# vsois/hanabi-agents

Hardware: AMD Instinct MI355X
Metric: env_steps_per_sec (higher is better)
Workload: dtype u8 env/encoder + bfloat16 Q-net GEMM (fp32 accumulate, fp32 master weights)

## Files before the change

### hanabi-agents_amd/csrc/actor_fused.hip

```cpp
#include <hip/hip_runtime.h>
#include <hip/hip_bf16.h>
#include <hip/hip_fp16.h>

#include <cstdint>

#include "../../include/hanabi_hip.h"
#include "common.hpp"
#include "env_kernel.hpp"

using hb::fail;

namespace {

typedef __bf16 bf16x8 __attribute__((ext_vector_type(8)));
typedef _Float16 f16x8 __attribute__((ext_vector_type(8)));
typedef float f32x4 __attribute__((ext_vector_type(4)));

constexpr int FM = 128;
constexpr int FH = 512;
constexpr int FNT = 512;
constexpr int FK = 51;
constexpr int S2 = FH / 32;
constexpr int LUT_BYTES = 65536;
constexpr int H_BYTES = FM * FH * 2;
constexpr int FRAG_FLOATS = 3 * 8 * FM;
constexpr int LDS_TOTAL = H_BYTES + FRAG_FLOATS * 4;
constexpr float NEG_BIG = -1e30f;

struct FusedArgs {
  const uint32_t* obs;
  long long m;
  int words;
  int s1;
  const uint4* w1f;
  const float* b1;
  const uint4* w2f;
  const float* b2;
  const float* support;
  float* q;
  int n_actions, n_pass;
  const int8_t* legal;
  int32_t* actions;
  float epsilon;
  unsigned long long seed, draw;
  long long first_gid;
  unsigned long long* stamps;
};

#ifdef HB_STAMPS
#define HB_FSTAMP(slot)                                                                              \
  do {                                                                                               \
    __builtin_amdgcn_sched_barrier(0);                                                               \
    unsigned long long hb_t_;                                                                        \
    asm volatile("s_memtime %0\n\ts_waitcnt lgkmcnt(0)" : "=s"(hb_t_)::"memory");                    \
    if (a.stamps && lane == 0) a.stamps[(static_cast<long long>(blockIdx.x) * 8 + wave) * 16 + (slot)] = hb_t_; \
    __builtin_amdgcn_sched_barrier(0);                                                               \
  } while (0)
#define HB_FSTAMP_REAL(slot)                                                                         \
  do {                                                                                               \
    unsigned long long hb_t_;                                                                        \
    asm volatile("s_memrealtime %0\n\ts_waitcnt lgkmcnt(0)" : "=s"(hb_t_)::"memory");                \
    if (a.stamps && lane == 0) a.stamps[(static_cast<long long>(blockIdx.x) * 8 + wave) * 16 + (slot)] = hb_t_; \
  } while (0)
#else
#define HB_FSTAMP(slot) do {} while (0)
#define HB_FSTAMP_REAL(slot) do {} while (0)
#endif

template <bool F16>
__device__ __forceinline__ uint32_t pack16(float lo, float hi) {
  if constexpr (F16) {
    const _Float16 a = static_cast<_Float16>(lo), b = static_cast<_Float16>(hi);
    uint16_t ua, ub;
    __builtin_memcpy(&ua, &a, 2);
    __builtin_memcpy(&ub, &b, 2);
    return static_cast<uint32_t>(ua) | (static_cast<uint32_t>(ub) << 16);
  } else {
    const __hip_bfloat16 a = __float2bfloat16(lo), b = __float2bfloat16(hi);
    return static_cast<uint32_t>(*reinterpret_cast<const uint16_t*>(&a)) |
           (static_cast<uint32_t>(*reinterpret_cast<const uint16_t*>(&b)) << 16);
  }
}
template <bool F16>
__device__ __forceinline__ uint32_t bits2_one(uint32_t b, int p) {
  const uint32_t t = (b >> (2 * p)) & 3u;
  return __umul24((t | (t << 15)) & 0x00010001u, F16 ? 0x3C00u : 0x3F80u);
}
template <bool F16>
__device__ __forceinline__ f32x4 mfma16(const uint4& wv, const uint4& xv, const f32x4& c) {
  if constexpr (F16) {
    union { uint4 u; f16x8 f; } w, x;
    w.u = wv; x.u = xv;
    return __builtin_amdgcn_mfma_f32_16x16x32_f16(w.f, x.f, c, 0, 0, 0);
  } else {
    union { uint4 u; bf16x8 f; } w, x;
    w.u = wv; x.u = xv;
    return __builtin_amdgcn_mfma_f32_16x16x32_bf16(w.f, x.f, c, 0, 0, 0);
  }
}
typedef float f32x2 __attribute__((ext_vector_type(2)));
typedef unsigned int u32x2 __attribute__((ext_vector_type(2)));
__device__ __forceinline__ float vmax(float a, float b) {
  float r;
  asm("v_max_f32 %0, %1, %2" : "=v"(r) : "v"(a), "v"(b));
  return r;
}
__device__ __forceinline__ float vmax3(float a, float b, float c) {
  float r;
  asm("v_max3_f32 %0, %1, %2, %3" : "=v"(r) : "v"(a), "v"(b), "v"(c));
  return r;
}
__device__ __forceinline__ float exp2_fast(float x) { return __builtin_amdgcn_exp2f(x); }

template <bool F16>
__global__ __launch_bounds__(FNT) void actor_fused_kernel(const FusedArgs a) {
  __shared__ __attribute__((aligned(16))) unsigned char lds[LDS_TOTAL];
  const int tid = threadIdx.x, lane = tid & 63;
  const int wave = __builtin_amdgcn_readfirstlane(tid >> 6);
  const int r = lane & 15, qd = lane >> 4;
  const long long row0 = static_cast<long long>(blockIdx.x) * FM;
  const int s1 = a.s1, G = (s1 + 3) >> 2;
  unsigned char* lutb = lds + (LDS_TOTAL - LUT_BYTES);
  const int bits_off = LDS_TOTAL - LUT_BYTES - 2048 * G;
  unsigned char* bits = lds + bits_off;
  const int m_early = bits_off >> 14;

  HB_FSTAMP_REAL(14);
  HB_FSTAMP(0);
  const uint4* w1p = a.w1f + (4 * wave) * 64 + lane;
  uint4 wa[4], wb[4];
#pragma unroll
  for (int n = 0; n < 4; ++n) wa[n] = w1p[n * 64];

  uint32_t w[4] = {0u, 0u, 0u, 0u};
  auto load_item = [&](int it) {
    const int rr = it & (FM - 1), g = it >> 7;
    long long row = row0 + rr;
    if (row >= a.m) row = a.m - 1;
    const uint32_t* src = a.obs + row * a.words + 4 * g;
#pragma unroll
    for (int i = 0; i < 4; ++i) w[i] = (4 * g + i < a.words) ? src[i] : 0u;
  };
  if (tid < FM * G) load_item(tid);
  for (int e = tid; e < 4096; e += FNT) {
    const uint32_t v = static_cast<uint32_t>(e) >> 4;
    *reinterpret_cast<uint4*>(lutb + e * 16) = make_uint4(bits2_one<F16>(v, 0), bits2_one<F16>(v, 1), bits2_one<F16>(v, 2), bits2_one<F16>(v, 3));
  }
  for (int it = tid; it < FM * G; it += FNT) {
    const int rr = it & (FM - 1), g = it >> 7;
    if (it != tid) load_item(it);
    uint32_t* dst = reinterpret_cast<uint32_t*>(bits) + (static_cast<size_t>((rr >> 4) * G + g) * 64 + (rr & 15));
#pragma unroll
    for (int qq = 0; qq < 4; ++qq) {
      const uint32_t o = ((w[0] >> (8 * qq)) & 0xFFu) | (((w[1] >> (8 * qq)) & 0xFFu) << 8) | (((w[2] >> (8 * qq)) & 0xFFu) << 16) |
                         (((w[3] >> (8 * qq)) & 0xFFu) << 24);
      dst[qq * 16] = o;
    }
  }
  HB_FSTAMP(1);
  __syncthreads();
  HB_FSTAMP(2);

  f32x4 acc[4][8];
#pragma unroll
  for (int n = 0; n < 4; ++n) {
    const float4 b = *reinterpret_cast<const float4*>(a.b1 + 64 * wave + 16 * n + 4 * qd);
#pragma unroll
    for (int m = 0; m < 8; ++m) acc[n][m] = f32x4{b.x, b.y, b.z, b.w};
  }

  {
    const unsigned char* lut = lutb + r * 16;
    const uint32_t* bw = reinterpret_cast<const uint32_t*>(bits) + lane;
#define HB_L1_STEP(I, WCUR, WNXT, HAVE_NEXT)                                                                   \
  {                                                                                                            \
    const int s_ = 4 * g + (I);                                                                                \
    if (HAVE_NEXT) {                                                                                           \
      _Pragma("unroll") for (int n = 0; n < 4; ++n) WNXT[n] = w1p[(s_ + 1) * 2048 + n * 64];                    \
    }                                                                                                          \
    asm volatile("" ::: "memory");                \
    uint4 xf[8];                                                                                               \
    _Pragma("unroll") for (int m = 0; m < 8; ++m) {                                                            \
      const uint32_t v = (xw[m] >> (8 * (I))) & 0xFFu;                                                         \
      xf[m] = *reinterpret_cast<const uint4*>(lut + v * 256u);                                                 \
    }                                                                                                          \
    _Pragma("unroll") for (int n = 0; n < 4; ++n) {                                                            \
      _Pragma("unroll") for (int m = 0; m < 8; ++m)                                                            \
        acc[n][m] = mfma16<F16>(WCUR[n], xf[m], acc[n][m]);                                                    \
    }                                                                                                          \
  }
    for (int g = 0; g < G; ++g) {
      uint32_t xw[8];
#pragma unroll
      for (int m = 0; m < 8; ++m) xw[m] = bw[(m * G + g) * 64];
      HB_L1_STEP(0, wa, wb, true)
      const bool more = 4 * g + 2 < s1;
      HB_L1_STEP(1, wb, wa, more)
      if (more) {
// ... 180 lines not shown
#pragma unroll
    HB_M HB_SWAP16(zs[m], HB_ADD)
#pragma unroll
    HB_M HB_SWAP16(zt[m], HB_ADD)
#pragma unroll
    HB_M HB_SWAP32(sF[m], HB_ADD)
#pragma unroll
    HB_M HB_SWAP32(tF[m], HB_ADD)
#pragma unroll
    HB_M HB_SWAP32(zs[m], HB_ADD)
#pragma unroll
    HB_M HB_SWAP32(zt[m], HB_ADD)
#pragma unroll
    HB_M { zm[m] = -nmz[m]; qF[m] = tF[m] * __builtin_amdgcn_rcpf(sF[m]) * (1.0f / FK); }
#undef HB_M
#undef HB_SWAP16
#undef HB_SWAP32
#undef HB_ADD
    if (qd == 0) {
#pragma unroll
      for (int m = 0; m < 4; ++m) {
        const long long row = row0 + 16 * (M0 + m) + r;
        if (full_ok && row < a.m) a.q[row * A + slot] = qF[m];
        fb[16 * (M0 + m) + r] = zm[m];
        fb[8 * FM + 16 * (M0 + m) + r] = zs[m];
        fb[16 * FM + 16 * (M0 + m) + r] = zt[m];
      }
    }
    __builtin_amdgcn_sched_barrier(0);
    });
    if (p < 2) HB_FSTAMP(8 + 3 * p);
    __syncthreads();
    if (tid < 2 * FM) {
      const int rr = tid & (FM - 1), g = tid >> 7;
      const int ea = full_cap + 2 * p + g;
      const long long row = row0 + rr;
      if (ea < A && row < a.m) {
        const float* f = reinterpret_cast<const float*>(lds + H_BYTES) + (4 * g) * FM + rr;
        const float m0 = f[0], m1 = f[FM], m2 = f[2 * FM], m3 = f[3 * FM];
        const float M = fmaxf(fmaxf(m0, m1), fmaxf(m2, m3));
        const float e0 = exp2_fast(m0 - M), e1 = exp2_fast(m1 - M), e2 = exp2_fast(m2 - M), e3 = exp2_fast(m3 - M);
        const float* fs = f + 8 * FM;
        const float* ft = f + 16 * FM;
        const float S = fs[0] * e0 + fs[FM] * e1 + fs[2 * FM] * e2 + fs[3 * FM] * e3;
        const float T = ft[0] * e0 + ft[FM] * e1 + ft[2 * FM] * e2 + ft[3 * FM] * e3;
        a.q[row * A + ea] = T * __builtin_amdgcn_rcpf(S) * (1.0f / FK);
      }
    }
    if (p + 1 < n_pass) __syncthreads();
    if (p < 2) HB_FSTAMP(9 + 3 * p);
  }
  if (a.legal) {
    asm volatile("s_waitcnt vmcnt(0)" ::: "memory");
    __syncthreads();
    if (tid < FM && row0 + tid < a.m) {
      const long long g = row0 + tid;
      const unsigned long long gid = static_cast<unsigned long long>(a.first_gid + g);
      uint32_t rnd[4];
      hb::philox4x32_10(static_cast<uint32_t>(a.draw), static_cast<uint32_t>(a.draw >> 32), static_cast<uint32_t>(gid),
                        static_cast<uint32_t>(gid >> 32), static_cast<uint32_t>(a.seed), static_cast<uint32_t>(a.seed >> 32), rnd);
      const float* qr = a.q + g * A;
      const int8_t* lr = a.legal + g * A;
      float best = -INFINITY;
      unsigned long long legal_mask = 0, ties = 0;
      for (int i = 0; i < A; ++i) {
        const float v = __hip_atomic_load(qr + i, __ATOMIC_RELAXED, __HIP_MEMORY_SCOPE_AGENT);
        if (lr[i] != 0) {
          legal_mask |= 1ull << i;
          if (v > best) { best = v; ties = 1ull << i; }
          else if (v == best) ties |= 1ull << i;
        }
      }
      const float u = static_cast<float>(rnd[0] >> 8) * (1.0f / 16777216.0f);
      unsigned long long pool = (u < a.epsilon) ? legal_mask : ties;
      if (pool == 0) pool = legal_mask;
      int pick = 0;
      const int c = __popcll(pool);
      if (c > 0) {
        int k = static_cast<int>(__umulhi(rnd[1], static_cast<uint32_t>(c)));
        while (k-- > 0) pool &= pool - 1;
        pick = __ffsll(static_cast<long long>(pool)) - 1;
      }
      a.actions[g] = pick;
    }
  }
  HB_FSTAMP_REAL(15);
}

struct PackArgs {
  const __hip_bfloat16* w1; int w1_ld;
  const __hip_bfloat16* b1;
  const __hip_bfloat16* w2; int w2_ld;
  const __hip_bfloat16* b2;
  int obs_len, s1, n_actions, n_pass;
  uint4* w1f; float* b1f; uint4* w2f; float* b2f;
  int chunks1, chunks2;
  int f16;
  uint16_t* w1t; int w1t_ld;
  uint16_t* w2t; int w2t_ld;
};
__device__ __forceinline__ float bias_to_float(const __hip_bfloat16* b, int i, int f16) {
  return f16 ? __half2float(reinterpret_cast<const __half*>(b)[i]) : __bfloat162float(b[i]);
}
__host__ __device__ __forceinline__ int fused_logit(int col, int n_actions, int n_pass) {
  const int slot = col >> 6, c = col & 63, n = c >> 4, q = (c >> 2) & 3, j = c & 3;
  const int r16 = 4 * n + j;
  const int full_cap = 8 * n_pass;
  int action, atom;
  if (r16 < 12 || (r16 == 12 && q < 3)) {
    action = slot < full_cap ? slot : n_actions;
    if (action >= n_actions) return -1;
    atom = r16 < 12 ? 4 * r16 + q : 48 + q;
  } else {
    const int p = slot >> 3, w = slot & 7, f = w & 3;
    action = full_cap + 2 * p + (w >> 2);
    atom = r16 == 12 ? 13 * f + 12 : 13 * f + 4 * (r16 - 13) + q;
  }
  if (action >= n_actions || atom >= FK) return -1;
  return action * FK + atom;
}
__global__ __launch_bounds__(256) void actor_fused_pack_kernel(const PackArgs a) {
  const int id = static_cast<int>(blockIdx.x) * 256 + static_cast<int>(threadIdx.x);
  const __hip_bfloat16 zero = __float2bfloat16(0.f);
  if (id < a.chunks1) {
    const int lane = id & 63, nt = (id >> 6) & 31, s = id >> 11;
    const int unit = 16 * nt + (lane & 15), k0 = 32 * s + 8 * (lane >> 4);
    __hip_bfloat16 v[8];
#pragma unroll
    for (int i = 0; i < 8; ++i) v[i] = (k0 + i < a.obs_len) ? a.w1[static_cast<long long>(k0 + i) * a.w1_ld + unit] : zero;
    a.w1f[id] = *reinterpret_cast<const uint4*>(v);
    if (a.w1t) *reinterpret_cast<uint4*>(a.w1t + static_cast<size_t>(unit) * a.w1t_ld + k0) = *reinterpret_cast<const uint4*>(v);
    if (id < FH) a.b1f[id] = bias_to_float(a.b1, id, a.f16);
  } else if (id < a.chunks1 + a.chunks2) {
    const int id2 = id - a.chunks1;
    const int lane = id2 & 63, ntp = (id2 >> 6) & 31, s = (id2 >> 11) % S2, pass = (id2 >> 11) / S2;
    const int col = 16 * (32 * pass + ntp) + (lane & 15), k0 = 32 * s + 8 * (lane >> 4);
    const int lg = fused_logit(col, a.n_actions, a.n_pass);
    __hip_bfloat16 v[8];
#pragma unroll
    for (int i = 0; i < 8; ++i) v[i] = lg >= 0 ? a.w2[static_cast<long long>(k0 + i) * a.w2_ld + lg] : zero;
    a.w2f[id2] = *reinterpret_cast<const uint4*>(v);
    if (a.w2t && lg >= 0) *reinterpret_cast<uint4*>(a.w2t + static_cast<size_t>(lg) * a.w2t_ld + k0) = *reinterpret_cast<const uint4*>(v);
    if (s == 0 && (lane >> 4) == 0) a.b2f[col] = lg >= 0 ? bias_to_float(a.b2, lg, a.f16) : NEG_BIG;
  }
}

bool aligned16(const void* p) { return (reinterpret_cast<uintptr_t>(p) & 15u) == 0; }
int passes_for(int n_actions) { return (n_actions + 9) / 10; }

}

extern "C" {

int hb_actor_fused_supported(int32_t obs_len, int32_t hidden, int32_t n_actions, int32_t n_atoms) {
  return obs_len >= 1 && obs_len <= 4096 && hidden == FH && n_atoms == FK && n_actions >= 1 && n_actions <= 80 ? 1 : 0;
}

int hb_actor_fused_columns(int32_t n_actions, int32_t* phys_of_logit_host) {
  if (!phys_of_logit_host) return fail(HB_ERR_INVALID, "null argument");
  if (n_actions < 1 || n_actions > 80) return fail(HB_ERR_INVALID, "n_actions must be 1..80");
  const int np = passes_for(n_actions);
  for (int j = 0; j < n_actions * FK; ++j) phys_of_logit_host[j] = -1;
  for (int col = 0; col < 512 * np; ++col) {
    const int lg = fused_logit(col, n_actions, np);
    if (lg >= 0) phys_of_logit_host[lg] = col;
  }
  for (int j = 0; j < n_actions * FK; ++j)
    if (phys_of_logit_host[j] < 0) return fail(HB_ERR_INVALID, "internal: logit column %d has no physical column", j);
  return HB_OK;
// ... 21 lines not shown
                             void* w2f_dev, float* b2f_dev, void* w1t_dev, int32_t w1t_ld, void* w2t_dev, int32_t w2t_ld,
                             int32_t dtype, void* stream) {
  if (dtype != 1 && dtype != 2) return fail(HB_ERR_INVALID, "dtype must be 1 (bf16) or 2 (f16)");
  if (!w1_dev || !b1_dev || !w2_dev || !b2_dev || !w1f_dev || !b1f_dev || !w2f_dev || !b2f_dev) return fail(HB_ERR_INVALID, "null argument");
  if (!hb_actor_fused_supported(obs_len, hidden, n_actions, n_atoms)) return fail(HB_ERR_INVALID, "shape not covered by the fused actor kernel");
  if (w1_ld < hidden || w2_ld < n_actions * n_atoms) return fail(HB_ERR_INVALID, "row strides shorter than the rows");
  if (!aligned16(w1f_dev) || !aligned16(w2f_dev)) return fail(HB_ERR_ALIGN, "w1f / w2f must be 16-byte aligned");
  PackArgs p{};
  p.w1 = static_cast<const __hip_bfloat16*>(w1_dev); p.w1_ld = w1_ld; p.b1 = static_cast<const __hip_bfloat16*>(b1_dev);
  p.w2 = static_cast<const __hip_bfloat16*>(w2_dev); p.w2_ld = w2_ld; p.b2 = static_cast<const __hip_bfloat16*>(b2_dev);
  p.obs_len = obs_len; p.s1 = 2 * ((obs_len + 63) / 64); p.n_actions = n_actions; p.n_pass = passes_for(n_actions);
  p.w1f = static_cast<uint4*>(w1f_dev); p.b1f = b1f_dev; p.w2f = static_cast<uint4*>(w2f_dev); p.b2f = b2f_dev;
  p.chunks1 = 32 * p.s1 * 64; p.chunks2 = 32 * p.n_pass * S2 * 64;
  p.f16 = dtype == 2 ? 1 : 0;
  if (w1t_dev && (w1t_ld < 32 * p.s1 || w1t_ld % 8 || !aligned16(w1t_dev))) return fail(HB_ERR_INVALID, "w1t: row stride must cover the padded K (a multiple of 8), 16-byte aligned");
  if (w2t_dev && (w2t_ld < hidden || w2t_ld % 8 || !aligned16(w2t_dev))) return fail(HB_ERR_INVALID, "w2t: row stride must cover the hidden units (a multiple of 8), 16-byte aligned");
  p.w1t = static_cast<uint16_t*>(w1t_dev); p.w1t_ld = w1t_ld; p.w2t = static_cast<uint16_t*>(w2t_dev); p.w2t_ld = w2t_ld;
  const int blocks = (p.chunks1 + p.chunks2 + 255) / 256;
  hipLaunchKernelGGL(actor_fused_pack_kernel, dim3(blocks), dim3(256), 0, static_cast<hipStream_t>(stream), p);
  HB_HIP(hipGetLastError());
  return HB_OK;
}

int hb_actor_fused_pack(const void* w1_dev, int32_t w1_ld, const void* b1_dev, const void* w2_dev, int32_t w2_ld, const void* b2_dev,
                        int32_t obs_len, int32_t hidden, int32_t n_actions, int32_t n_atoms, void* w1f_dev, float* b1f_dev, void* w2f_dev,
                        float* b2f_dev, void* stream) {
  return hb_actor_fused_pack_dt(w1_dev, w1_ld, b1_dev, w2_dev, w2_ld, b2_dev, obs_len, hidden, n_actions, n_atoms, w1f_dev, b1f_dev,
                                w2f_dev, b2f_dev, 1, stream);
}

struct FusedSelect {
  const int8_t* legal;
  int32_t* actions;
  float epsilon;
  uint64_t seed, draw;
  int64_t first_gid;
};
static int fused_launch(const uint32_t* obs_bits_dev, int64_t n_rows, int32_t obs_len, const void* w1f_dev, const float* b1f_dev,
                        const void* w2f_dev, const float* b2f_dev, const float* support_dev, int32_t hidden, int32_t n_actions,
                        int32_t n_atoms, float* q_dev, unsigned long long* stamps_dev, const FusedSelect* sel, int32_t dtype, void* stream);

int hb_actor_fused_q_dt(const uint32_t* obs_bits_dev, int64_t n_rows, int32_t obs_len, const void* w1f_dev, const float* b1f_dev,
                        const void* w2f_dev, const float* b2f_dev, const float* support_dev, int32_t hidden, int32_t n_actions,
                        int32_t n_atoms, float* q_dev, int32_t dtype, void* stream) {
  return fused_launch(obs_bits_dev, n_rows, obs_len, w1f_dev, b1f_dev, w2f_dev, b2f_dev, support_dev, hidden, n_actions, n_atoms, q_dev,
                      nullptr, nullptr, dtype, stream);
}

int hb_actor_fused_act_dt(const uint32_t* obs_bits_dev, const int8_t* legal_dev, int64_t n_rows, int32_t obs_len, const void* w1f_dev,
                          const float* b1f_dev, const void* w2f_dev, const float* b2f_dev, const float* support_dev, int32_t hidden,
                          int32_t n_actions, int32_t n_atoms, float* q_dev, float epsilon, uint64_t seed, uint64_t draw,
                          int64_t first_game_id, int32_t* actions_dev, int32_t dtype, void* stream) {
  if (!legal_dev || !actions_dev) return fail(HB_ERR_INVALID, "null argument");
  if (n_actions > 64) return fail(HB_ERR_INVALID, "n_actions must be 1..64 for the fused selection");
  const FusedSelect sel{legal_dev, actions_dev, epsilon, seed, draw, first_game_id};
  return fused_launch(obs_bits_dev, n_rows, obs_len, w1f_dev, b1f_dev, w2f_dev, b2f_dev, support_dev, hidden, n_actions, n_atoms, q_dev,
                      nullptr, &sel, dtype, stream);
}

int hb_actor_fused_q(const uint32_t* obs_bits_dev, int64_t n_rows, int32_t obs_len, const void* w1f_dev, const float* b1f_dev,
                     const void* w2f_dev, const float* b2f_dev, const float* support_dev, int32_t hidden, int32_t n_actions, int32_t n_atoms,
                     float* q_dev, void* stream) {
  return fused_launch(obs_bits_dev, n_rows, obs_len, w1f_dev, b1f_dev, w2f_dev, b2f_dev, support_dev, hidden, n_actions, n_atoms, q_dev,
                      nullptr, nullptr, 1, stream);
}

int hb_actor_fused_act(const uint32_t* obs_bits_dev, const int8_t* legal_dev, int64_t n_rows, int32_t obs_len, const void* w1f_dev,
                       const float* b1f_dev, const void* w2f_dev, const float* b2f_dev, const float* support_dev, int32_t hidden,
                       int32_t n_actions, int32_t n_atoms, float* q_dev, float epsilon, uint64_t seed, uint64_t draw,
                       int64_t first_game_id, int32_t* actions_dev, void* stream) {
  return hb_actor_fused_act_dt(obs_bits_dev, legal_dev, n_rows, obs_len, w1f_dev, b1f_dev, w2f_dev, b2f_dev, support_dev, hidden,
                               n_actions, n_atoms, q_dev, epsilon, seed, draw, first_game_id, actions_dev, 1, stream);
}

#ifdef HB_STAMPS
int hb_actor_fused_q_stamped(const uint32_t* obs_bits_dev, int64_t n_rows, int32_t obs_len, const void* w1f_dev, const float* b1f_dev,
                             const void* w2f_dev, const float* b2f_dev, const float* support_dev, int32_t hidden, int32_t n_actions,
                             int32_t n_atoms, float* q_dev, unsigned long long* stamps_dev, void* stream) {
  return fused_launch(obs_bits_dev, n_rows, obs_len, w1f_dev, b1f_dev, w2f_dev, b2f_dev, support_dev, hidden, n_actions, n_atoms, q_dev,
                      stamps_dev, nullptr, 1, stream);
}
#endif

static int fused_launch(const uint32_t* obs_bits_dev, int64_t n_rows, int32_t obs_len, const void* w1f_dev, const float* b1f_dev,
                        const void* w2f_dev, const float* b2f_dev, const float* support_dev, int32_t hidden, int32_t n_actions,
                        int32_t n_atoms, float* q_dev, unsigned long long* stamps_dev, const FusedSelect* sel, int32_t dtype, void* stream) {
  if (dtype != 1 && dtype != 2) return fail(HB_ERR_INVALID, "dtype must be 1 (bf16) or 2 (f16)");
  if (!obs_bits_dev || !w1f_dev || !b1f_dev || !w2f_dev || !b2f_dev || !support_dev || !q_dev) return fail(HB_ERR_INVALID, "null argument");
  if (!hb_actor_fused_supported(obs_len, hidden, n_actions, n_atoms)) return fail(HB_ERR_INVALID, "shape not covered by the fused actor kernel");
  if (n_rows <= 0) return HB_OK;
  if (!aligned16(w1f_dev) || !aligned16(w2f_dev) || !aligned16(b1f_dev) || !aligned16(b2f_dev))
    return fail(HB_ERR_ALIGN, "w1f / w2f / b1f / b2f must be 16-byte aligned");
  FusedArgs a{};
  a.obs = obs_bits_dev; a.m = n_rows; a.words = (obs_len + 31) / 32; a.s1 = 2 * ((obs_len + 63) / 64);
  a.w1f = static_cast<const uint4*>(w1f_dev); a.b1 = b1f_dev; a.w2f = static_cast<const uint4*>(w2f_dev); a.b2 = b2f_dev;
  a.support = support_dev; a.q = q_dev; a.n_actions = n_actions; a.n_pass = passes_for(n_actions);
  a.stamps = stamps_dev;
  if (sel) {
    a.legal = sel->legal; a.actions = sel->actions; a.epsilon = sel->epsilon; a.seed = sel->seed; a.draw = sel->draw;
    a.first_gid = sel->first_gid;
  }
  const dim3 grid(static_cast<unsigned>((n_rows + FM - 1) / FM));
  if (dtype == 2) hipLaunchKernelGGL(actor_fused_kernel<true>, grid, dim3(FNT), 0, static_cast<hipStream_t>(stream), a);
  else hipLaunchKernelGGL(actor_fused_kernel<false>, grid, dim3(FNT), 0, static_cast<hipStream_t>(stream), a);
  HB_HIP(hipGetLastError());
  return HB_OK;
}

}
```

### hanabi-agents_amd/csrc/chain.hip

```cpp
#include <hip/hip_runtime.h>

#include <cstdint>

#include "../../include/hanabi_hip.h"
#include "common.hpp"

using hb::fail;

extern "C" {

int hb_chain_run(const hb_cmd* cmds, int32_t count, const int64_t* vars_i, const double* vars_f) {
  if (!cmds || count < 0) return fail(HB_ERR_INVALID, "null argument");
  for (int32_t k = 0; k < count; ++k) {
    const hb_cmd& c = cmds[k];
    if (c.cond >= 0 && (!vars_i || vars_i[c.cond] == 0)) continue;
    const int64_t* vi = c.var >= 0 ? vars_i + c.var : nullptr;
    const double* vf = c.fvar >= 0 ? vars_f + c.fvar : nullptr;
    if ((c.var >= 0 && !vars_i) || (c.fvar >= 0 && !vars_f)) return fail(HB_ERR_INVALID, "command %d needs a variable array", k);
    int rc = HB_OK;
    switch (c.op) {
      case HB_CMD_WAIT_EVENT:
        rc = hb_stream_wait_event(c.stream, c.p[0]);
        break;
      case HB_CMD_RECORD_EVENT:
        rc = hb_event_record(c.p[0], c.stream);
        break;
      case HB_CMD_REPLAY_INSERT:
        if (!vi) return fail(HB_ERR_INVALID, "command %d: hb_replay_insert needs its start variable", k);
        rc = hb_replay_insert(static_cast<int8_t*>(c.p[0]), static_cast<const int8_t*>(c.p[1]), static_cast<const int8_t*>(c.p[2]),
                              static_cast<const int32_t*>(c.p[3]), static_cast<const float*>(c.p[4]),
                              static_cast<const int8_t*>(c.p[5]), static_cast<int8_t*>(c.p[6]), static_cast<int8_t*>(c.p[7]),
                              static_cast<int8_t*>(c.p[8]), static_cast<int8_t*>(c.p[9]), static_cast<float*>(c.p[10]),
                              static_cast<uint8_t*>(c.p[11]), c.i[0], static_cast<int32_t>(c.i[1]), static_cast<int32_t>(c.i[2]),
                              c.i[3], vi[0], c.stream);
        break;
      case HB_CMD_ACTOR_FUSED_ACT:
        if (!vi || !vf) return fail(HB_ERR_INVALID, "command %d: hb_actor_fused_act needs its draw and epsilon variables", k);
        rc = hb_actor_fused_act_dt(static_cast<const uint32_t*>(c.p[0]), static_cast<const int8_t*>(c.p[1]), c.i[0],
                                   static_cast<int32_t>(c.i[1]), c.p[2], static_cast<const float*>(c.p[3]), c.p[4],
                                   static_cast<const float*>(c.p[5]), static_cast<const float*>(c.p[6]), static_cast<int32_t>(c.i[2]),
                                   static_cast<int32_t>(c.i[3]), static_cast<int32_t>(c.i[4]), static_cast<float*>(c.p[7]),
                                   static_cast<float>(vf[0]), static_cast<uint64_t>(c.i[5]), static_cast<uint64_t>(vi[0]), c.i[6],
                                   static_cast<int32_t*>(c.p[8]), c.i[7] == 2 ? 2 : 1, c.stream);
        break;
      case HB_CMD_ENV_STEP_PACKED:
        rc = hb_env_step_packed(static_cast<hb_env*>(c.p[0]), static_cast<const int32_t*>(c.p[1]), static_cast<uint32_t*>(c.p[2]),
                                static_cast<int8_t*>(c.p[3]), static_cast<int8_t*>(c.p[4]), static_cast<float*>(c.p[5]),
                                static_cast<int8_t*>(c.p[6]), static_cast<float*>(c.p[7]), static_cast<int8_t*>(c.p[8]),
                                static_cast<int8_t*>(c.p[9]), c.stream);
        break;
      case HB_CMD_TREE_FILL_RANGE:
        if (!vi) return fail(HB_ERR_INVALID, "command %d: hb_tree_fill_range needs its range variables", k);
        if (vi[1] > 0) rc = hb_tree_fill_range(static_cast<hb_tree*>(c.p[0]), vi[0], vi[1], static_cast<const float*>(c.p[1]), c.stream);
        break;
      case HB_CMD_PER_SAMPLE_GATHER:
        rc = hb_per_sample_gather(static_cast<hb_tree*>(c.p[0]), static_cast<uint64_t>(c.i[0]), static_cast<const float*>(c.p[1]), c.i[1],
                                  static_cast<int64_t*>(c.p[2]), static_cast<double*>(c.p[3]), c.p[4], c.p[5],
                                  static_cast<const int8_t*>(c.p[6]), static_cast<const float*>(c.p[7]),
                                  static_cast<const uint8_t*>(c.p[8]), static_cast<int32_t>(c.i[2]), static_cast<int32_t>(c.i[3]), c.p[9],
                                  static_cast<int32_t>(c.i[4]), static_cast<int32_t>(c.i[5]), static_cast<int32_t*>(c.p[10]),
                                  static_cast<float*>(c.p[11]), static_cast<float*>(c.p[12]), static_cast<float*>(c.p[13]),
                                  static_cast<int32_t>(c.i[6]), static_cast<float>(c.f[0]), c.i[7], c.i[8],
                                  static_cast<const int64_t*>(c.p[14]), c.stream);
        break;
      case HB_CMD_GRAPH_LAUNCH:
        if (!c.p[0]) return fail(HB_ERR_INVALID, "command %d: null graph", k);
        HB_HIP(hipGraphLaunch(static_cast<hipGraphExec_t>(c.p[0]), static_cast<hipStream_t>(c.stream)));
        break;
      case HB_CMD_PER_UPDATE:
        rc = hb_per_update(static_cast<hb_tree*>(c.p[0]), static_cast<const int64_t*>(c.p[1]), static_cast<const float*>(c.p[2]), c.i[0],
                           c.f[0], static_cast<float*>(c.p[3]), static_cast<float*>(c.p[4]), c.stream);
        break;
      case HB_CMD_ACTOR_FUSED_PACK:
        rc = hb_actor_fused_pack_thin(c.p[0], static_cast<int32_t>(c.i[0]), c.p[1], c.p[2], static_cast<int32_t>(c.i[1]), c.p[3],
                                      static_cast<int32_t>(c.i[2]), static_cast<int32_t>(c.i[3]), static_cast<int32_t>(c.i[4]),
                                      static_cast<int32_t>(c.i[5]), c.p[4], static_cast<float*>(c.p[5]), c.p[6], static_cast<float*>(c.p[7]),
                                      c.p[8], static_cast<int32_t>(c.i[7]), c.p[9], static_cast<int32_t>(c.i[8]), c.i[6] == 2 ? 2 : 1, c.stream);
        break;
      case HB_CMD_ACTOR_PACK_WEIGHTS:
        rc = hb_actor_pack_weights(static_cast<const hb_pack_job*>(c.p[0]), static_cast<int32_t>(c.i[0]), c.stream);
        break;
      default:
        return fail(HB_ERR_INVALID, "command %d: unknown op %d", k, c.op);
    }
    if (rc != HB_OK) return rc;
  }
  return HB_OK;
}

}
```

### hanabi-agents_amd/csrc/env_api.hip

```cpp
#include <hip/hip_runtime.h>

#include <cstdarg>
#include <cstdio>
#include <cstdlib>
#include <cstring>
#include <new>
#include <string>
#include <vector>

#include "../../include/hanabi_hip.h"
#include "common.hpp"
#include "env_kernel.hpp"

namespace hb {
const EnvVariant* variants_full(int* n);
const EnvVariant* variants_small(int* n);
const EnvVariant* variants_vsmall(int* n);

thread_local std::string g_error;
int fail(int code, const char* fmt, ...) {
  char buf[512];
  va_list ap;
  va_start(ap, fmt);
  vsnprintf(buf, sizeof buf, fmt, ap);
// ... 123 lines not shown
}

int hb_env_destroy(hb_env* e) {
  if (!e) return HB_OK;
  if (e->state) (void)hipFree(e->state);
  if (e->illegal) (void)hipFree(e->illegal);
  if (e->next_deck) (void)hipFree(e->next_deck);
  if (e->refill) (void)hipFree(e->refill);
  if (e->side) { (void)hipStreamSynchronize(e->side); (void)hipStreamDestroy(e->side); }
  if (e->ev_step_done) (void)hipEventDestroy(e->ev_step_done);
  if (e->ev_refill_done) (void)hipEventDestroy(e->ev_refill_done);
  delete e;
  return HB_OK;
}

int64_t hb_env_num_games(const hb_env* e) { return e ? e->n : 0; }

int hb_env_set_decks(hb_env* e, const uint8_t* decks_dev) {
  if (!e) return fail(HB_ERR_INVALID, "null env");
  e->decks = decks_dev;
  e->refill_in_flight = false;
  HB_HIP(hipDeviceSynchronize());
  HB_HIP(hipMemset(e->refill, 1, static_cast<size_t>(e->n)));
  return HB_OK;
}

int hb_env_set_games_per_wave(hb_env* e, int32_t g) {
  if (!e) return fail(HB_ERR_INVALID, "null env");
  if (g != 0 && g != 8 && g != 16 && g != 32 && g != 64)
    return fail(HB_ERR_INVALID, "games per wave must be 0 (automatic), 8, 16, 32 or 64");
  e->gpw = g;
  return HB_OK;
}

int hb_env_set_profile_events(hb_env* e, void* start_event, void* stop_event) {
  if (!e) return fail(HB_ERR_INVALID, "null env");
  if ((start_event == nullptr) != (stop_event == nullptr)) return fail(HB_ERR_INVALID, "pass both events or neither");
  e->ev_start = static_cast<hipEvent_t>(start_event);
  e->ev_stop = static_cast<hipEvent_t>(stop_event);
  return HB_OK;
}

static void fill_common(hb_env* e, hb::EnvArgs& a) {
  a.state = e->state;
  a.decks = e->decks;
  a.next_deck = e->next_deck;
  a.refill = e->refill;
  a.illegal = e->illegal;
  a.stats = e->illegal + 1;
  a.n = e->n;
  a.seed = e->seed;
  a.first_gid = e->first_gid;
  a.flags = e->cfg.flags;
}

static int join_refill(hb_env* e, void* stream) {
  if (e->refill_in_flight) {
    HB_HIP(hipStreamWaitEvent(static_cast<hipStream_t>(stream), e->ev_refill_done, 0));
    e->refill_in_flight = false;
  }
  return HB_OK;
}

static int refill(hb_env* e, void* stream) {
  e->since_refill = 0;
  hb::EnvArgs a{};
  fill_common(e, a);
  e->var->refill(a, static_cast<hipStream_t>(stream));
  HB_HIP(hipGetLastError());
  return HB_OK;
}

static int refill_async(hb_env* e, void* stream) {
  if (++e->since_refill < e->refill_period) return HB_OK;
  if (!e->async_refill) return refill(e, stream);
  HB_HIP(hipEventRecord(e->ev_step_done, static_cast<hipStream_t>(stream)));
  HB_HIP(hipStreamWaitEvent(e->side, e->ev_step_done, 0));
  if (int rc = refill(e, e->side)) return rc;
  HB_HIP(hipEventRecord(e->ev_refill_done, e->side));
  e->refill_in_flight = true;
  return HB_OK;
}

static int launch(hb_env* e, hb::EnvArgs& a, void* stream) {
  a.state = e->state;
  a.decks = e->decks;
  a.next_deck = e->next_deck;
  a.refill = e->refill;
  a.illegal = e->illegal;
  a.stats = e->illegal + 1;
  a.n = e->n;
  a.seed = e->seed;
  a.first_gid = e->first_gid;
  a.flags = e->cfg.flags;
  {
    static const int always = [] { const char* v = getenv("HB_ENV_DECK_ALWAYS"); return v && v[0] == '1' ? 0x100 : 0; }();
    a.flags |= always;
  }
  a.ev_start = e->ev_start;
  a.ev_stop = e->ev_stop;
  const int gpw = e->gpw ? e->gpw : ((a.obs_bits && !a.obs && e->n >= 32768) ? 32 : 16);
  hb::LaunchFn fn = gpw == 8 ? e->var->g8 : (gpw == 16 ? e->var->g16 : (gpw == 32 ? e->var->g32 : e->var->g64));
  fn(a, static_cast<hipStream_t>(stream));
  HB_HIP(hipGetLastError());
  return HB_OK;
}

static int check_out(const void* obs, const void* legal) {
  if (!obs || !legal) return fail(HB_ERR_INVALID, "obs_dev and legal_dev are required");
  if ((reinterpret_cast<uintptr_t>(obs) & 15) || (reinterpret_cast<uintptr_t>(legal) & 15))
    return fail(HB_ERR_ALIGN, "obs_dev / legal_dev must be 16-byte aligned");
  return HB_OK;
}
static int check_out_packed(const void* bits, const void* obs, const void* legal) {
  if (!bits || !legal) return fail(HB_ERR_INVALID, "obs_bits_dev and legal_dev are required");
  if ((reinterpret_cast<uintptr_t>(bits) & 15) || (reinterpret_cast<uintptr_t>(legal) & 15) || (reinterpret_cast<uintptr_t>(obs) & 15))
    return fail(HB_ERR_ALIGN, "obs_bits_dev / obs_dev / legal_dev must be 16-byte aligned");
  return HB_OK;
}

int hb_env_reset(hb_env* e, const uint8_t* mask_dev, int32_t start_player, void* stream) {
  if (!e) return fail(HB_ERR_INVALID, "null env");
  if (start_player < 0 || start_player >= e->cfg.players) return fail(HB_ERR_INVALID, "start_player out of range");
  hb::EnvArgs a{};
  a.mode = hb::MODE_RESET;
  a.mask = mask_dev;
  a.start_player = start_player;
  if (int rc = join_refill(e, stream)) return rc;
  if (int rc = refill(e, stream)) return rc;
  if (int rc = launch(e, a, stream)) return rc;
  return refill(e, stream);
}

int hb_env_observe(hb_env* e, int8_t* obs_dev, int8_t* legal_dev, float* agent_reward_dev, int8_t* agent_step_type_dev,
                   void* stream) {
  if (!e) return fail(HB_ERR_INVALID, "null env");
  if (int rc = check_out(obs_dev, legal_dev)) return rc;
  hb::EnvArgs a{};
  a.mode = hb::MODE_OBSERVE;
  a.obs = obs_dev;
  a.legal = legal_dev;
  a.agent_reward = agent_reward_dev;
  a.agent_step_type = agent_step_type_dev;
  return launch(e, a, stream);
}

int hb_env_step(hb_env* e, const int32_t* actions_dev, int8_t* obs_dev, int8_t* legal_dev, float* reward_dev,
                int8_t* terminal_dev, float* agent_reward_dev, int8_t* agent_step_type_dev, int8_t* score_dev,
                void* stream) {
  if (!e) return fail(HB_ERR_INVALID, "null env");
  if (!actions_dev) return fail(HB_ERR_INVALID, "actions_dev is required");
  if (int rc = check_out(obs_dev, legal_dev)) return rc;
  hb::EnvArgs a{};
  a.mode = hb::MODE_STEP;
  a.actions = actions_dev;
  a.obs = obs_dev;
  a.legal = legal_dev;
  a.reward = reward_dev;
  a.terminal = terminal_dev;
  a.agent_reward = agent_reward_dev;
  a.agent_step_type = agent_step_type_dev;
  a.score = score_dev;
  if (int rc = join_refill(e, stream)) return rc;
  if (int rc = launch(e, a, stream)) return rc;
  return refill_async(e, stream);
}

int hb_env_observe_packed(hb_env* e, uint32_t* obs_bits_dev, int8_t* obs_dev, int8_t* legal_dev, float* agent_reward_dev,
                          int8_t* agent_step_type_dev, void* stream) {
  if (!e) return fail(HB_ERR_INVALID, "null env");
  if (int rc = check_out_packed(obs_bits_dev, obs_dev, legal_dev)) return rc;
  hb::EnvArgs a{};
  a.mode = hb::MODE_OBSERVE;
  a.obs = obs_dev;
  a.obs_bits = obs_bits_dev;
  a.legal = legal_dev;
  a.agent_reward = agent_reward_dev;
  a.agent_step_type = agent_step_type_dev;
  return launch(e, a, stream);
}

int hb_env_step_packed(hb_env* e, const int32_t* actions_dev, uint32_t* obs_bits_dev, int8_t* obs_dev, int8_t* legal_dev,
                       float* reward_dev, int8_t* terminal_dev, float* agent_reward_dev, int8_t* agent_step_type_dev,
                       int8_t* score_dev, void* stream) {
  if (!e) return fail(HB_ERR_INVALID, "null env");
  if (!actions_dev) return fail(HB_ERR_INVALID, "actions_dev is required");
  if (int rc = check_out_packed(obs_bits_dev, obs_dev, legal_dev)) return rc;
  hb::EnvArgs a{};
  a.mode = hb::MODE_STEP;
  a.actions = actions_dev;
  a.obs = obs_dev;
  a.obs_bits = obs_bits_dev;
  a.legal = legal_dev;
  a.reward = reward_dev;
  a.terminal = terminal_dev;
  a.agent_reward = agent_reward_dev;
  a.agent_step_type = agent_step_type_dev;
  a.score = score_dev;
  if (int rc = join_refill(e, stream)) return rc;
  if (int rc = launch(e, a, stream)) return rc;
  return refill_async(e, stream);
}

int hb_env_step_select_packed(hb_env* e, const float* q_dev, const int8_t* sel_legal_dev, float epsilon, uint64_t seed, uint64_t draw,
                              int64_t first_game_id, int32_t* actions_out_dev, uint32_t* obs_bits_dev, int8_t* obs_dev,
                              int8_t* legal_dev, float* reward_dev, int8_t* terminal_dev, float* agent_reward_dev,
                              int8_t* agent_step_type_dev, int8_t* score_dev, void* stream) {
  if (!e) return fail(HB_ERR_INVALID, "null env");
  if (!q_dev || !sel_legal_dev || !actions_out_dev) return fail(HB_ERR_INVALID, "q_dev, sel_legal_dev and actions_out_dev are required");
  if ((reinterpret_cast<uintptr_t>(q_dev) & 15) || (reinterpret_cast<uintptr_t>(sel_legal_dev) & 3))
    return fail(HB_ERR_ALIGN, "q_dev must be 16-byte and sel_legal_dev 4-byte aligned");
  if (e->var->n_actions > 64) return fail(HB_ERR_INVALID, "the fused selection handles at most 64 actions");
  if (int rc = check_out_packed(obs_bits_dev, obs_dev, legal_dev)) return rc;
  hb::EnvArgs a{};
  a.mode = hb::MODE_STEP;
  a.sel_q = q_dev;
  a.sel_legal = sel_legal_dev;
  a.sel_actions = actions_out_dev;
  a.sel_eps = epsilon;
  a.sel_seed = seed;
  a.sel_draw = draw;
  a.sel_first_gid = first_game_id;
  a.obs = obs_dev;
  a.obs_bits = obs_bits_dev;
  a.legal = legal_dev;
  a.reward = reward_dev;
  a.terminal = terminal_dev;
  a.agent_reward = agent_reward_dev;
  a.agent_step_type = agent_step_type_dev;
  a.score = score_dev;
  if (int rc = join_refill(e, stream)) return rc;
  if (int rc = launch(e, a, stream)) return rc;
  return refill_async(e, stream);
}

#ifdef HB_STAMPS
int hb_env_step_stamped(hb_env* e, const int32_t* actions_dev, int8_t* obs_dev, int8_t* legal_dev,
                        unsigned long long* stamps_dev, void* stream) {
  hb::EnvArgs a{};
  a.mode = hb::MODE_STEP;
  a.actions = actions_dev;
  a.obs = obs_dev;
  a.legal = legal_dev;
  a.stamps = stamps_dev;
  if (int rc = join_refill(e, stream)) return rc;
  if (int rc = launch(e, a, stream)) return rc;
  return refill_async(e, stream);
}
#endif

int hb_env_illegal_count(hb_env* e, int64_t* out) {
  if (!e || !out) return fail(HB_ERR_INVALID, "null argument");
  unsigned long long v = 0;
  HB_HIP(hipMemcpy(&v, e->illegal, 8, hipMemcpyDeviceToHost));
  *out = static_cast<int64_t>(v);
  return HB_OK;
}

int hb_env_stats(hb_env* e, int64_t* episodes, int64_t* score_sum) {
  if (!e || !episodes || !score_sum) return fail(HB_ERR_INVALID, "null argument");
  std::vector<unsigned long long> v(static_cast<size_t>(2 * e->stat_slots));
  HB_HIP(hipMemcpy(v.data(), e->illegal + 1, 16 * e->stat_slots, hipMemcpyDeviceToHost));
  unsigned long long ep = 0, sc = 0;
  for (long long i = 0; i < e->stat_slots; ++i) { ep += v[2 * i]; sc += v[2 * i + 1]; }
  *episodes = static_cast<int64_t>(ep);
  *score_sum = static_cast<int64_t>(sc);
  return HB_OK;
}

int hb_env_set_refill_period(hb_env* e, int32_t steps) {
  if (!e) return fail(HB_ERR_INVALID, "null env");
  if (steps < 1 || steps > e->cfg.max_life) return fail(HB_ERR_INVALID, "refill period must be 1..max_life (%d)", e->cfg.max_life);
  e->refill_period = steps;
  return HB_OK;
}

int hb_env_set_async_refill(hb_env* e, int32_t on) {
  if (!e) return fail(HB_ERR_INVALID, "null env");
  HB_HIP(hipDeviceSynchronize());
  e->refill_in_flight = false;
  e->async_refill = on != 0;
  return HB_OK;
}

int hb_env_export_state(hb_env* e, uint32_t* rows_dev, void* stream) {
  if (!e || !rows_dev) return fail(HB_ERR_INVALID, "null argument");
  HB_HIP(hipMemcpyAsync(rows_dev, e->state, static_cast<size_t>(e->n) * e->var->state_words * 4, hipMemcpyDeviceToDevice,
                        static_cast<hipStream_t>(stream)));
  return HB_OK;
}
const uint32_t* hb_env_state(hb_env* e) { return e ? e->state : nullptr; }

int hb_env_import_state(hb_env* e, const uint32_t* rows_dev, void* stream) {
  if (!e || !rows_dev) return fail(HB_ERR_INVALID, "null argument");
  HB_HIP(hipMemcpyAsync(e->state, rows_dev, static_cast<size_t>(e->n) * e->var->state_words * 4, hipMemcpyDeviceToDevice,
                        static_cast<hipStream_t>(stream)));
  if (int rc = join_refill(e, stream)) return rc;
  HB_HIP(hipMemsetAsync(e->refill, 1, static_cast<size_t>(e->n), static_cast<hipStream_t>(stream)));
  return refill(e, stream);
}

__global__ void random_legal_kernel(const int8_t* __restrict__ legal, long long n, int n_actions, unsigned long long seed,
                                    unsigned long long draw, long long first_gid, int32_t* __restrict__ actions) {
  const long long g = static_cast<long long>(blockIdx.x) * blockDim.x + threadIdx.x;
  if (g >= n) return;
  const unsigned long long gid = static_cast<unsigned long long>(first_gid + g);
  uint32_t out[4];
  hb::philox4x32_10(static_cast<uint32_t>(draw), static_cast<uint32_t>(draw >> 32), static_cast<uint32_t>(gid),
                    static_cast<uint32_t>(gid >> 32), static_cast<uint32_t>(seed), static_cast<uint32_t>(seed >> 32), out);
  const int8_t* row = legal + g * n_actions;
  unsigned long long m = 0;
  for (int i = 0; i < n_actions; ++i) m |= static_cast<unsigned long long>(row[i] != 0) << i;
  const int n_legal = __popcll(m);
  int pick = 0;
  if (n_legal > 0) {
    int k = static_cast<int>(__umulhi(out[0], static_cast<uint32_t>(n_legal)));
    while (k-- > 0) m &= m - 1;
// ... 43 lines not shown
```

### hanabi-agents_amd/csrc/env_kernel.hpp

```cpp
#pragma once
#include <hip/hip_runtime.h>
#include <hip/hip_ext.h>
#include <stdint.h>
#include <utility>

namespace hb {

enum { MODE_STEP = 0, MODE_OBSERVE = 1, MODE_RESET = 2 };
constexpr int NEXT_DECK_BYTES = 64;
enum { MV_PLAY = 0, MV_DISCARD = 1, MV_RCOLOR = 2, MV_RRANK = 3 };

struct EnvArgs {
  uint32_t* state;
  const int32_t* actions;
  const uint8_t* mask;
  const uint8_t* decks;
  uint8_t* next_deck;
  uint8_t* refill;
  int8_t* obs;
  uint32_t* obs_bits;
  int8_t* legal;
  float* reward;
  int8_t* terminal;
  float* agent_reward;
  int8_t* agent_step_type;
  int8_t* score;
  unsigned long long* illegal;
  unsigned long long* stats;
  long long n;
  unsigned long long seed;
  long long first_gid;
  int flags;
  int mode;
  int start_player;
  const float* sel_q;
  const int8_t* sel_legal;
  int32_t* sel_actions;
  float sel_eps;
  unsigned long long sel_seed, sel_draw;
  long long sel_first_gid;
  unsigned long long* stamps;
  hipEvent_t ev_start, ev_stop;
};

#ifdef HB_STAMPS
#define HB_STAMP(slot)                                                                               \
  do {                                                                                               \
    __builtin_amdgcn_sched_barrier(0);                                                               \
    unsigned long long hb_t_;                                                                        \
    asm volatile("s_memtime %0\n\ts_waitcnt lgkmcnt(0)" : "=s"(hb_t_)::"memory");                    \
    __builtin_amdgcn_sched_barrier(0);                                                               \
    if (a.stamps && lane == 0) a.stamps[(static_cast<long long>(blockIdx.x) * 4 + wave) * 12 + (slot)] = hb_t_; \
  } while (0)
#define HB_STAMP_REAL(slot)                                                                          \
  do {                                                                                               \
    if (a.stamps && lane == 0)                                                                       \
      a.stamps[(static_cast<long long>(blockIdx.x) * 4 + wave) * 12 + (slot)] = __builtin_amdgcn_s_memrealtime(); \
  } while (0)
#else
#define HB_STAMP(slot) do { } while (0)
#define HB_STAMP_REAL(slot) do { } while (0)
#endif

template <int P_, int C_, int R_, int H_, int INFO_, int LIFE_>
struct Cfg {
  static constexpr int P = P_, C = C_, R = R_, H = H_, INFO = INFO_, LIFE = LIFE_;
  static constexpr int BITS = C * R;
  static constexpr int copies(int r) { return r == 0 ? 3 : (r == R - 1 ? 1 : 2); }
  static constexpr int cum(int r) {
    int s = 0;
    for (int i = 0; i < r; ++i) s += copies(i);
    return s;
  }
  static constexpr int CPC = cum(R);
  static constexpr int D = C * CPC;
  static constexpr int A = 2 * H + (P - 1) * (C + R);
  static constexpr int FLAGS_OFF = (P - 1) * H * BITS;
  static constexpr int BOARD_OFF = FLAGS_OFF + P;
  static constexpr int DECK_T = D - P * H;
  static constexpr int FW_OFF = BOARD_OFF + DECK_T;
  static constexpr int INFO_OFF = FW_OFF + BITS;
  static constexpr int LIFE_OFF = INFO_OFF + INFO;
  static constexpr int DISC_OFF = LIFE_OFF + LIFE;
  static constexpr int LA_OFF = DISC_OFF + D;
  static constexpr int LA_LEN = P + 4 + P + C + R + H + H + BITS + 2;
  static constexpr int KN_OFF = LA_OFF + LA_LEN;
  static constexpr int KN_SLOT = BITS + C + R;
  static constexpr int OBS_LEN = KN_OFF + P * H * KN_SLOT;
  static constexpr int NW = (OBS_LEN + 31) / 32;
  static constexpr int NWP = (NW + 1) | 1;
  static constexpr int LW = 3;
  static constexpr int SW = P <= 3 ? 32 : 48;
  static constexpr int SWP = SW + 1;
  static constexpr int W_HANDS = 10, W_KNOW = 10 + P, W_DECK = 10 + 3 * P;
  static constexpr uint32_t ALL_PLAUSIBLE = ((1u << C) - 1u) | (((1u << R) - 1u) << 5);
  static_assert(W_DECK * 4 + D <= SW * 4, "state row too small");
  static_assert(BITS <= 25 && D <= 50 && A <= 64 && H <= 5 && P <= 5 && INFO <= 15 && LIFE <= 7, "limits");
};

template <class F, int... Is>
__device__ __forceinline__ void static_for_impl(F&& f, std::integer_sequence<int, Is...>) {
  (f(std::integral_constant<int, Is>{}), ...);
}
template <int N, class F>
__device__ __forceinline__ void static_for(F&& f) {
  static_for_impl(static_cast<F&&>(f), std::make_integer_sequence<int, N>{});
}

template <int C, int R>
__device__ __forceinline__ uint32_t spread_colors(uint32_t cp) {
  if constexpr (2 * (R - 1) >= C && C * R <= 24 + 1) {
    constexpr auto sum = [](int first, int step) constexpr {
      uint32_t v = 0;
      for (int k = first; k < C; k += 2) v |= 1u << (step * k);
      return v;
    };
    constexpr uint32_t EIN = sum(0, 1), OIN = sum(1, 1), EMUL = sum(0, R - 1), OMUL = sum(1, R - 1), ESEL = sum(0, R),
                       OSEL = sum(1, R);
    uint32_t v = __umul24(cp & EIN, EMUL) & ESEL;
    if constexpr (C > 1) v |= __umul24(cp & OIN, OMUL) & OSEL;
    return v;
  } else {
    uint32_t v = 0;
#pragma unroll
    for (int c = 0; c < C; ++c) v |= ((cp >> c) & 1u) << (c * R);
    return v;
  }
}

template <int NW>
struct BitAcc {
  uint32_t w[NW];
  __device__ __forceinline__ void clear() {
#pragma unroll
    for (int i = 0; i < NW; ++i) w[i] = 0;
  }
  template <int OFF, int LEN>
  __device__ __forceinline__ void put(uint32_t v) {
    static_assert(LEN >= 0 && LEN <= 32 && OFF >= 0 && (OFF + LEN + 31) / 32 <= NW, "put range");
    if constexpr (LEN > 0) {
// ... 51 lines not shown
        l += Rm;
        if (l >= CPR) { l -= CPR; ++g; }
      }
#pragma unroll
      for (int u = 0; u < 4; ++u) {
        if (c0 + 64 * u < chunks) {
          u32x4 o;
          o.x = spread4(v[u]);
          o.y = spread4(v[u] >> 4);
          o.z = spread4(v[u] >> 8);
          o.w = spread4(v[u] >> 12);
          __builtin_nontemporal_store(o, reinterpret_cast<u32x4_unaligned*>(out + off[u]));
        }
      }
    }
  }
  if constexpr (TAIL > 0) {
    const int n = nvalid * TAIL;
    for (int e = lane; e < n; e += 64) {
      const int g = e / TAIL, j = e - g * TAIL, k = CPR * 16 + j;
      out[g * L + k] = static_cast<int8_t>((bits[g * row_stride + (k >> 5)] >> (k & 31)) & 1u);
    }
  }
}

template <int A>
__device__ __forceinline__ int select_action(const EnvArgs& a, long long gi) {
  float qv[A];
  uint32_t lw[(A + 3) / 4];
  const float* qr = a.sel_q + gi * A;
  const int8_t* lr = a.sel_legal + gi * A;
  if constexpr (A % 4 == 0) {
#pragma unroll
    for (int i = 0; i < A / 4; ++i) {
      const float4 v = reinterpret_cast<const float4*>(qr)[i];
      qv[4 * i] = v.x; qv[4 * i + 1] = v.y; qv[4 * i + 2] = v.z; qv[4 * i + 3] = v.w;
      lw[i] = reinterpret_cast<const uint32_t*>(lr)[i];
    }
  } else {
#pragma unroll
    for (int i = 0; i < (A + 3) / 4; ++i) lw[i] = 0;
#pragma unroll
    for (int i = 0; i < A; ++i) {
      qv[i] = qr[i];
      lw[i >> 2] |= static_cast<uint32_t>(static_cast<uint8_t>(lr[i])) << (8 * (i & 3));
    }
  }
  const unsigned long long gid = static_cast<unsigned long long>(a.sel_first_gid + gi);
  uint32_t r[4];
  philox4x32_10(static_cast<uint32_t>(a.sel_draw), static_cast<uint32_t>(a.sel_draw >> 32), static_cast<uint32_t>(gid),
                static_cast<uint32_t>(gid >> 32), static_cast<uint32_t>(a.sel_seed), static_cast<uint32_t>(a.sel_seed >> 32), r);
  float best = -INFINITY;
  unsigned long long legal_mask = 0, ties = 0;
#pragma unroll
  for (int i = 0; i < A; ++i) {
    const float v = qv[i];
    if ((lw[i >> 2] >> (8 * (i & 3))) & 0xFFu) {
      legal_mask |= 1ull << i;
      if (v > best) { best = v; ties = 1ull << i; }
      else if (v == best) ties |= 1ull << i;
    }
  }
  const float u = static_cast<float>(r[0] >> 8) * (1.0f / 16777216.0f);
  unsigned long long pool = (u < a.sel_eps) ? legal_mask : ties;
  if (pool == 0) pool = legal_mask;
  int pick = 0;
  const int c = __popcll(pool);
  if (c > 0) {
    int k = static_cast<int>(__umulhi(r[1], static_cast<uint32_t>(c)));
    while (k-- > 0) pool &= pool - 1;
    pick = __ffsll(static_cast<long long>(pool)) - 1;
  }
  a.sel_actions[gi] = pick;
  return pick;
}

__device__ __forceinline__ void wave_sync() {
  __builtin_amdgcn_fence(__ATOMIC_RELEASE, "wavefront");
  __builtin_amdgcn_wave_barrier();
  __builtin_amdgcn_fence(__ATOMIC_ACQUIRE, "wavefront");
}

template <class K, int G>
__global__ __launch_bounds__(256) void env_kernel(const EnvArgs a) {
  constexpr int P = K::P, C = K::C, R = K::R, H = K::H;
  constexpr int LPG = 1;
  constexpr int PER_WAVE = G * (K::SWP + K::NWP + K::LW);
  __shared__ uint32_t lds[4 * PER_WAVE];

  const int lane = threadIdx.x & 63;
  const int wave = threadIdx.x >> 6;
  uint32_t* const srow = lds + wave * PER_WAVE;
  uint32_t* const obits = srow + G * K::SWP;
  uint32_t* const lbits = obits + G * K::NWP;
  const long long g0 = (static_cast<long long>(blockIdx.x) * 4 + wave) * G;
  const long long left = a.n - g0;
  const int nvalid = left <= 0 ? 0 : (left < G ? static_cast<int>(left) : G);
  const int mode = a.mode;
  HB_STAMP_REAL(10);
  HB_STAMP(0);

  const bool active = lane < nvalid && lane < G;
  const long long gi = g0 + lane;
  int uid_in = 0;
  bool mask_in = true;
  uint4 nd[4] = {make_uint4(0u, 0u, 0u, 0u), make_uint4(0u, 0u, 0u, 0u), make_uint4(0u, 0u, 0u, 0u), make_uint4(0u, 0u, 0u, 0u)};
  const uint4* const ndp = reinterpret_cast<const uint4*>(a.next_deck + gi * NEXT_DECK_BYTES);
  if (active) {
    if (mode == MODE_STEP) uid_in = a.sel_q ? select_action<K::A>(a, gi) : a.actions[gi];
    if (mode == MODE_RESET && a.mask) mask_in = a.mask[gi] != 0;
    if ((mode == MODE_RESET && mask_in) || (mode == MODE_STEP && (a.flags & 0x100))) {
      nd[0] = ndp[0]; nd[1] = ndp[1]; nd[2] = ndp[2]; nd[3] = ndp[3];
    }
  }

  {
    constexpr int Q = K::SW / 4;
    constexpr int ROUNDS = (G * Q + 63) / 64;
    const uint4* src = reinterpret_cast<const uint4*>(a.state + g0 * K::SW);
    uint4 v[ROUNDS];
#pragma unroll
    for (int r = 0; r < ROUNDS; ++r) {
      const int e = lane + 64 * r;
      v[r] = e < nvalid * Q ? src[e] : make_uint4(0u, 0u, 0u, 0u);
    }
#pragma unroll
    for (int r = 0; r < ROUNDS; ++r) {
      const int e = lane + 64 * r;
      if (e < nvalid * Q) {
        const int g = e / Q, q = e - g * Q;
        uint32_t* d = srow + g * K::SWP + 4 * q;
        d[0] = v[r].x; d[1] = v[r].y; d[2] = v[r].z; d[3] = v[r].w;
      }
    }
  }
  HB_STAMP(1);
  wave_sync();
  HB_STAMP(2);

  uint32_t* const row = srow + lane * K::SWP;
  uint32_t w0 = 0, w1 = 0, w2 = 0, w3 = 0, w6 = 0;
  uint64_t accw = 0, disc = 0;
  float out_reward = 0.f;
  int out_term = 0, out_score = 0;
  bool illegal = false, need_reset = false, keep_seats = true;
  int reset_start = 0;

  auto hand_n = [&](int p) -> int { return (w1 >> (15 + 3 * p)) & 7; };
  auto fw = [&](int c) -> int { return (w1 >> (3 * c)) & 7; };
  auto score_now = [&]() -> int {
    if (((w0 >> 10) & 7) == 0) return 0;
    int s = 0;
#pragma unroll
    for (int c = 0; c < C; ++c) s += fw(c);
    return s;
  };

  if (active) {
    w0 = row[0]; w1 = row[1]; w2 = row[2]; w3 = row[3]; w6 = row[6];
    accw = (static_cast<uint64_t>(row[5]) << 32) | row[4];
    disc = (static_cast<uint64_t>(row[9]) << 32) | row[8];
    if (mode == MODE_RESET) {
      need_reset = mask_in;
      keep_seats = false;
      reset_start = a.start_player;
    } else if (mode == MODE_STEP && ((w0 >> 19) & 3) == 0) {
      {
        int fsum = 0;
#pragma unroll
        for (int c = 0; c < C; ++c) fsum += fw(c);
        if (!(a.flags & 0x100) && (((w0 >> 10) & 7) <= 1 || (w0 & 63) == 0 || fsum >= C * R - 1)) {
          nd[0] = ndp[0]; nd[1] = ndp[1]; nd[2] = ndp[2]; nd[3] = ndp[3];
        }
      }
      const int deck_size = w0 & 63, info = (w0 >> 6) & 15, life = (w0 >> 10) & 7;
      const int s = (w0 >> 13) & 7;
      const int turns = (w0 >> 16) & 7, moves = (w0 >> 21) & 255;
      const bool in_range = uid_in >= 0 && uid_in < K::A;
      const int uid = in_range ? uid_in : 0;
      const bool is_discard = uid < H, is_play = uid >= H && uid < 2 * H;
      const bool is_rc = uid >= 2 * H && uid < 2 * H + (P - 1) * C, is_rr = uid >= 2 * H + (P - 1) * C;
      const bool card_move = is_discard || is_play, is_hint = !card_move;
      const int type = is_play ? MV_PLAY : (is_discard ? MV_DISCARD : (is_rc ? MV_RCOLOR : MV_RRANK));
      const int xc = uid - 2 * H, xr = uid - 2 * H - (P - 1) * C;
      const int ci = is_discard ? uid : (is_play ? uid - H : 0);
      const int toff = is_rc ? 1 + xc / C : (is_rr ? 1 + xr / R : 0);
      const int hcol = is_rc ? xc % C : 0, hrank = is_rr ? xr % R : 0;
      int t = s + toff;
      if (t >= P) t -= P;
      const int n_s = hand_n(s), n_t = hand_n(t);
      const uint32_t hs = row[K::W_HANDS + s], ht = row[K::W_HANDS + t];
      const uint64_t kn_s = (static_cast<uint64_t>(row[K::W_KNOW + 2 * s + 1]) << 32) | row[K::W_KNOW + 2 * s];
// ... 175 lines not shown
        const uint32_t own = (1u << n_o) - 1u;
        if (info < K::INFO) legal |= own;
        legal |= static_cast<uint64_t>(own) << H;
        acc.template put64<K::BOARD_OFF, K::DECK_T>((1ull << deck_size) - 1ull);
        static_for<C>([&](auto CI) {
          constexpr int c = decltype(CI)::value;
          acc.template put<K::FW_OFF + c * R, R>((1u << fw(c)) >> 1);
        });
        acc.template put<K::INFO_OFF, K::INFO>((1u << info) - 1u);
        acc.template put<K::LIFE_OFF, K::LIFE>((1u << life) - 1u);
        acc.template put64<K::DISC_OFF, K::D>(disc);
        {
          const uint32_t valid = w2 & 1u;
          const int la_player = (w2 >> 1) & 7, la_type = (w2 >> 4) & 3, la_ci = (w2 >> 6) & 7, la_toff = (w2 >> 9) & 7;
          const int la_color = (w2 >> 12) & 7, la_rank = (w2 >> 15) & 7;
          const uint32_t la_scored = (w2 >> 18) & 1u, la_info = (w2 >> 19) & 1u, la_mask = (w2 >> 20) & 31u;
          int actor = la_player - o;
          if (actor < 0) actor += P;
          int target = actor + la_toff;
          if (target >= P) target -= P;
          const uint32_t reveal = valid & static_cast<uint32_t>(la_type >= MV_RCOLOR);
          const uint32_t cardmv = valid & static_cast<uint32_t>(la_type <= MV_DISCARD);
          const uint32_t is_rc = valid & static_cast<uint32_t>(la_type == MV_RCOLOR);
          const uint32_t is_rr = valid & static_cast<uint32_t>(la_type == MV_RRANK);
          const uint32_t is_play = valid & static_cast<uint32_t>(la_type == MV_PLAY);
          constexpr int o1 = K::LA_OFF, o2 = o1 + P, o3 = o2 + 4, o4 = o3 + P, o5 = o4 + C, o6 = o5 + R, o7 = o6 + H,
                        o8 = o7 + H, o9 = o8 + K::BITS;
          acc.template put<o1, P>(valid << actor);
          acc.template put<o2, 4>(valid << la_type);
          acc.template put<o3, P>(reveal << target);
          acc.template put<o4, C>(is_rc << la_color);
          acc.template put<o5, R>(is_rr << la_rank);
          acc.template put<o6, H>(reveal ? la_mask : 0u);
          acc.template put<o7, H>(cardmv << la_ci);
          acc.template put<o8, K::BITS>(cardmv << (la_color * R + la_rank));
          acc.template put<o9, 2>((is_play & la_scored) | ((is_play & la_info) << 1));
        }
        static_for<P>([&](auto REL) {
          constexpr int rel = decltype(REL)::value;
          int p = o + rel;
          if (p >= P) p -= P;
          const int n_p = hand_n(p);
          const uint64_t kn = (static_cast<uint64_t>(row[K::W_KNOW + 2 * p + 1]) << 32) | row[K::W_KNOW + 2 * p];
          static_for<H>([&](auto I) {
            constexpr int i = decltype(I)::value;
            const uint32_t k = static_cast<uint32_t>(kn >> (12 * i)) & 0xFFFu;
            const uint32_t cp = k & 31u, rp = (k >> 5) & 31u;
            const uint32_t plaus = __umul24(spread_colors<C, R>(cp), rp);
            const uint32_t ch = (k >> 10) & 1u, rh = (k >> 11) & 1u;
            uint64_t v = plaus | (static_cast<uint64_t>(ch ? cp : 0u) << K::BITS) |
                         (static_cast<uint64_t>(rh ? rp : 0u) << (K::BITS + C));
            if (i >= n_p) v = 0;
            acc.template put64<K::KN_OFF + (rel * H + i) * K::KN_SLOT, K::KN_SLOT>(v);
          });
        });
        uint32_t* ob = obits + lane * K::NWP;
  #pragma unroll
        for (int i = 0; i < K::NW; ++i) ob[i] = acc.w[i];
  #pragma unroll
        for (int i = K::NW; i < K::NWP; ++i) ob[i] = 0;
        uint32_t* lb = lbits + lane * K::LW;
        lb[0] = static_cast<uint32_t>(legal);
        lb[1] = static_cast<uint32_t>(legal >> 32);
        lb[2] = 0;
      }
      const uint32_t pend = (w3 >> o) & 1u, tsin = (w3 >> (5 + o)) & 1u;
      if (a.agent_reward) a.agent_reward[gi] = pend ? static_cast<float>(static_cast<int8_t>(accw >> (8 * o))) : 0.f;
      if (a.agent_step_type) a.agent_step_type[gi] = static_cast<int8_t>(!pend ? 0 : (tsin ? 2 : 1));
      if (mode == MODE_STEP) {
        if (a.reward) a.reward[gi] = out_reward;
        if (a.terminal) a.terminal[gi] = static_cast<int8_t>(out_term);
        if (a.score) a.score[gi] = static_cast<int8_t>(out_score);
      }
    }
  }
  if (mode == MODE_STEP) {
    const unsigned long long bad = __ballot(illegal);
    if (bad && lane == 0) atomicAdd(a.illegal, static_cast<unsigned long long>(__popcll(bad)));
    const unsigned long long ended = __ballot(out_term != 0);
    if (ended) {
      int sc = out_term ? out_score : 0;
      for (int o = 32; o > 0; o >>= 1) sc += __shfl_xor(sc, o);
      if (lane == 0) {
        unsigned long long* slot = a.stats + 2 * (static_cast<long long>(blockIdx.x) * 4 + wave);
        atomicAdd(slot, static_cast<unsigned long long>(__popcll(ended)));
        atomicAdd(slot + 1, static_cast<unsigned long long>(sc));
      }
    }
  }
  HB_STAMP(6);
  wave_sync();
  HB_STAMP(7);

  if (mode != MODE_OBSERVE) {
    constexpr int Q = K::SW / 4;
    uint4* dst = reinterpret_cast<uint4*>(a.state + g0 * K::SW);
    for (int e = lane; e < nvalid * Q; e += 64) {
      const int g = e / Q, q = e - g * Q;
      const uint32_t* s = srow + g * K::SWP + 4 * q;
      uint4 v;
      v.x = s[0]; v.y = s[1]; v.z = s[2]; v.w = s[3];
      dst[e] = v;
    }
  }
  HB_STAMP(8);
  if (mode != MODE_RESET) {
    if (a.obs_bits) {
      uint32_t* dst = a.obs_bits + g0 * K::NW;
      for (int e = lane; e < nvalid * K::NW; e += 64) {
        const int g = e / K::NW, i = e - g * K::NW;
        dst[e] = obits[g * K::NWP + i];
      }
    }
    if (a.obs) expand_rows<K::OBS_LEN>(obits, K::NWP, nvalid, a.obs + g0 * K::OBS_LEN, lane);
    expand_rows<K::A>(lbits, K::LW, nvalid, a.legal + g0 * K::A, lane);
  }
  HB_STAMP(9);
  HB_STAMP_REAL(11);
}

template <class K>
__global__ __launch_bounds__(256) void refill_kernel(const EnvArgs a) {
  constexpr int GR = 16;
  const int lane = threadIdx.x & 63;
  const long long g0 = (static_cast<long long>(blockIdx.x) * 4 + (threadIdx.x >> 6)) * GR;
  if (g0 >= a.n) return;
  const long long gi = g0 + lane;
  const bool mine = lane < GR && gi < a.n && a.refill[gi] != 0;
  unsigned long long todo = __ballot(mine);
  while (todo) {
    const int src = __ffsll(static_cast<long long>(todo)) - 1;
    todo &= todo - 1;
    const long long g = g0 + src;
    uint8_t* dst = a.next_deck + g * NEXT_DECK_BYTES;
    if (a.decks) {
      if (lane < K::D) dst[lane] = a.decks[g * K::D + lane];
    } else {
      const uint32_t episode = a.state[g * K::SW + 6];
      const unsigned long long gid = static_cast<unsigned long long>(a.first_gid + g);
      uint32_t out[4];
      philox4x32_10(static_cast<uint32_t>(lane), episode, static_cast<uint32_t>(gid), static_cast<uint32_t>(gid >> 32),
                    static_cast<uint32_t>(a.seed), static_cast<uint32_t>(a.seed >> 32), out);
      const uint32_t key = (out[0] & ~63u) | static_cast<uint32_t>(lane);
      int rank = 0;
      static_for<K::D>([&](auto I) {
        constexpr int i = decltype(I)::value;
        const uint32_t ki = static_cast<uint32_t>(__builtin_amdgcn_readlane(static_cast<int>(key), i));
        rank += ki < key ? 1 : 0;
      });
      if (lane < K::D) {
        const int col = lane / K::CPC, k = lane - col * K::CPC;
        const int rk = k < 3 ? 0 : 1 + (k - 3) / 2;
        dst[rank] = static_cast<uint8_t>(col * K::R + rk);
      }
    }
  }
  if (mine) a.refill[gi] = 0;
}

template <class K>
void launch_refill(const EnvArgs& a, hipStream_t stream) {
  const unsigned blocks = static_cast<unsigned>((a.n + 63) / 64);
  if (blocks == 0) return;
  hipLaunchKernelGGL((refill_kernel<K>), dim3(blocks), dim3(256), 0, stream, a);
}

template <class K, int G>
void launch_env(const EnvArgs& a, hipStream_t stream) {
  const long long per_block = 4LL * G;
  const unsigned blocks = static_cast<unsigned>((a.n + per_block - 1) / per_block);
  if (blocks == 0) return;
  if (a.ev_start && a.ev_stop)
    hipExtLaunchKernelGGL((env_kernel<K, G>), dim3(blocks), dim3(256), 0, stream, a.ev_start, a.ev_stop, 0, a);
  else
    hipLaunchKernelGGL((env_kernel<K, G>), dim3(blocks), dim3(256), 0, stream, a);
}

using LaunchFn = void (*)(const EnvArgs&, hipStream_t);
struct EnvVariant {
  int P, C, R, H, INFO, LIFE;
  int obs_len, n_actions, deck, state_words;
  LaunchFn g8, g16, g32, g64, refill;
};

template <class K>
constexpr EnvVariant make_variant() {
  return EnvVariant{K::P, K::C, K::R, K::H, K::INFO, K::LIFE, K::OBS_LEN, K::A, K::D, K::SW,
                    &launch_env<K, 8>, &launch_env<K, 16>, &launch_env<K, 32>, &launch_env<K, 64>, &launch_refill<K>};
}

}
```

### hanabi-agents_amd/hanabi_agents/rlax_dqn/fused_learner.py

```python
import os

import torch

from hanabi_hip import _capi as K

_DT = {torch.float32: 0, torch.bfloat16: 1, torch.float16: 2}


class FusedLearner:
    def __init__(self, agent):
        self.agent = agent
        p = agent.params
        dev = agent.device
        self.cd = {"float32": torch.float32, "bfloat16": torch.bfloat16, "float16": torch.float16}[p.compute_dtype]
        self.B = p.train_batch_size
        self.A, self.Kk = agent.atoms.shape
        self.L = agent.obs_len
        layers = agent.online.layers
        assert len(layers) == 2, "the fused learner covers the reference topology: one hidden layer (params.layers=[H])"
        self.layers = layers
        B, AK = self.B, self.A * self.Kk
        H = layers[0].out_features
        f32 = dict(dtype=torch.float32, device=dev)
        pad = (lambda v, m: (v + m - 1) // m * m) if self.cd != torch.float32 else (lambda v, m: v)
# ... 196 lines not shown
            K.check(L.hb_thin_gemm(K.dptr(hcat), K.dptr(self.w2stT), K.dptr(self.b2st), K.dptr(logits), 2 * B, self.Np, H, 2 * H, H,
                                   self.Np, 2, H, self.Np * H, 2 * B * self.Np, 2 | f16, s))
        else:
            hcat = torch._addmm_activation(self.b1cat, self.x, self.w1cat, use_gelu=False)
            logits = torch.bmm(hcat.view(2 * B, 2, H).transpose(0, 1), self.w2st)
        logits_on, logits_t = logits[0], logits[1, B:]
        hb, xb = hcat[:B, :H], self.x[:B]
        ldt = 0 if self.thin else _DT[self.cd]
        bon, btg = (None, None) if self.thin else (self.b2st[0], self.b2st[1])
        if self.sparse_backward:
            K.check(L.hb_c51_loss_sparse(K.dptr(logits_on), K.dptr(logits_t), ldt, K.dptr(self.act), K.dptr(self.rew),
                                         K.dptr(self.term), K.dptr(prios), K.dptr(a._beta), K.dptr(self.disc),
                                         1 if a.params.mask_terminal else 0, K.dptr(self.support), B, self.A, self.Kk, self.Np,
                                         K.dptr(self.td), K.dptr(self.w_is), K.dptr(self.dl), K.dptr(self.step),
                                         K.dptr(bon), K.dptr(btg), s))
            K.check(L.hb_c51_backward(K.dptr(self.dl), K.dptr(self.act), K.dptr(hb), hb.stride(0), K.dptr(w2), w2.stride(0),
                                      _DT[self.cd], B, H, self.A, self.Kk, K.dptr(self.dh), K.dptr(self.g_b1),
                                      K.dptr(self._gw2_out), self.Np, K.dptr(self._gb2_pad), s))
            dh = self.dh
        else:
            if self.thin:
                logits_on, logits_t, ldt = logits_on.to(self.cd), logits_t.to(self.cd), _DT[self.cd]
            K.check(L.hb_c51_loss_grad(K.dptr(logits_on), K.dptr(logits_t), ldt, K.dptr(self.act), K.dptr(self.rew),
                                       K.dptr(self.term), K.dptr(prios), K.dptr(a._beta), K.dptr(self.disc),
                                       1 if a.params.mask_terminal else 0, K.dptr(self.support), B, self.A, self.Kk, self.Np,
                                       K.dptr(self.td), K.dptr(self.w_is), K.dptr(self.dlogits), K.dptr(self.step),
                                       K.dptr(bon), K.dptr(btg), s))
            dl = self.dlogits
            torch.mm(hb.t(), dl, out=self._gw2_out)
            K.check(L.hb_colsum(K.dptr(dl), _DT[self.cd], B, self.Np, K.dptr(self._gb2_pad), s))
            dh = torch.mm(dl, w2.t())
            K.check(L.hb_relu_bwd_colsum(K.dptr(dh), K.dptr(hb), hb.stride(0), _DT[self.cd], B, dh.shape[1], K.dptr(self.g_b1), s))
        torch.mm(xb.t(), dh, out=self._gw1_out)
        if not self.direct:
            self.g_w2.copy_(self._gw2_out[:, :self.AK])
            self.g_b2.copy_(self._gb2_pad[:self.AK])
            self.g_w1.copy_(self._gw1_out[:self.L])
        return self.td, self.w_is

    def _adam_table(self):
        if self._adam_tab is None:
            if self.direct:
                grads = (((self._gw1_out, _DT[self.cd], self._gw1_out.shape[1]), (self.g_b1, 0, 0)),
                         ((self._gw2_out, _DT[self.cd], self.Np), (self._gb2_pad, 0, 0)))
            else:
                grads = (((self.g_w1, 0, 0), (self.g_b1, 0, 0)), ((self.g_w2, 0, 0), (self.g_b2, 0, 0)))
            tab = (K.HbAdamTensor * 4)()
            k = 0
            for li, l in enumerate(self.layers):
                for names, noise, g, eff in ((("w", "w_mu", "w_sigma"), l.eps_w, grads[li][0], self.eff[li][0]),
                                             (("b", "b_mu", "b_sigma"), l.eps_b, grads[li][1], self.eff[li][1])):
                    ps = [getattr(l, n) for n in names]
                    st = [self.state[(li, n)] for n in names]
                    d = tab[k]
                    d.w, d.w_mu, d.w_sigma = (p.data_ptr() for p in ps)
                    d.noise, d.grad, d.grad_dtype, d.grad_ld = noise.data_ptr(), g[0].data_ptr(), g[1], g[2]
                    d.m_w, d.v_w = st[0][0].data_ptr(), st[0][1].data_ptr()
                    d.m_mu, d.v_mu = st[1][0].data_ptr(), st[1][1].data_ptr()
                    d.m_sigma, d.v_sigma = st[2][0].data_ptr(), st[2][1].data_ptr()
                    d.eff, d.n, d.cols = eff.data_ptr(), ps[0].numel(), ps[0].shape[-1]
                    d.eff_ld = eff.stride(0) if eff.dim() == 2 else eff.shape[-1]
                    k += 1
            self._adam_tab = tab
        return self._adam_tab

    def _pack_table(self):
        if self._pack_tab is None:
            import ctypes

            n_log = self.A * self.Kk
            host = (ctypes.c_int32 * n_log)()
            K.check(K.lib().hb_actor_fused_columns(self.A, host))
            self._col_map = torch.tensor(list(host), dtype=torch.int32, device=self.agent.device)
            f = self.actor.fsets[0]
            tab = (K.HbAdamPack * 4)()
            tab[0].wt, tab[0].wt_ld, tab[0].frag, tab[0].frag_kind = self.w1catT.data_ptr(), self.Kp, f[0].data_ptr(), 1
            tab[1].bias_f32 = f[1].data_ptr()
            tab[2].wt, tab[2].wt_ld, tab[2].frag, tab[2].frag_kind = self.w2stT[0].data_ptr(), self.H, f[2].data_ptr(), 2
            tab[2].col_map_dev = self._col_map.data_ptr()
            tab[3].bias_f32, tab[3].col_map_dev = f[3].data_ptr(), self._col_map.data_ptr()
            self._pack_tab = tab
        return self._pack_tab

    def part2(self):
        p = self.agent.params
        if self.adam_pack:
            K.check(K.lib().hb_noisy_adam_multi_pack(self._adam_table(), self._pack_table(), 4, K.dptr(self.step), 0.0, _DT[self.cd],
                                                     float(p.learning_rate), 0.9, 0.999, 3.125e-5, K.current_stream()))
            self._packed_in_part2 = True
            return
        K.check(K.lib().hb_noisy_adam_multi(self._adam_table(), 4, K.dptr(self.step), 0.0, _DT[self.cd],
                                            float(p.learning_rate), 0.9, 0.999, 3.125e-5, K.current_stream()))
        self._packed_in_part2 = False
        if self.actor is not None and not self.lag:
            (w1, b1), (w2, b2) = self.eff
            self.actor.pack(w1, b1, w2, b2, 0, lazy_two_kernel=True, thin=self._thin_out())
            self._packed_in_part2 = True

    def loss(self):
        return torch.mean(self.td * self.w_is)
```

### hanabi-agents_amd/hanabi_agents/rlax_dqn/rlax_rainbow.py

```python
import os
from typing import Tuple

import numpy as np
import torch

from . import bitpack
from . import learning as L
from .experience_buffer import ExperienceBuffer
from .noisy_mlp import NoisyMLP, PlainMLP
from .params import RlaxRainbowParams
from .priority_buffer import PriorityBuffer

_DTYPES = {"float32": torch.float32, "bfloat16": torch.bfloat16, "float16": torch.float16}


def _shape_of(spec):
    return tuple(spec.shape)


class DQNPolicy:

    @staticmethod
    def q_values(network, atoms, obs, legal, distributional=True):
        out = network(obs)
# ... 55 lines not shown
    def __init__(self, observation_spec, action_spec, params: RlaxRainbowParams = RlaxRainbowParams(), device=None,
                 process_group=None, use_graphs=True, use_fused_learner=True):
        if not callable(params.epsilon):
            eps = params.epsilon
            params = params._replace(epsilon=lambda ts: eps)
        if not callable(params.beta_is):
            beta = params.beta_is
            params = params._replace(beta_is=lambda ts: beta)
        self.params = params
        self.device = torch.device(device) if device is not None else torch.device(
            "cuda" if torch.cuda.is_available() else "cpu")
        self.process_group = process_group
        n_games, obs_len = _shape_of(observation_spec)
        self.n_actions = int(action_spec.num_values)
        self.obs_len = obs_len
        cd = _DTYPES[params.compute_dtype]
        self.distributional = bool(params.distributional)

        def build():
            if self.distributional:
                return NoisyMLP(obs_len, tuple(params.layers) + (self.n_actions * params.n_atoms,), seed=params.seed,
                                compute_dtype=cd)
            return PlainMLP(obs_len, tuple(params.layers) + (self.n_actions,), seed=params.seed, compute_dtype=cd)

        self.online = build().to(self.device)
        self.target = build().to(self.device)
        self.target.load_state_dict(self.online.state_dict())
        for p in self.target.parameters():
            p.requires_grad_(False)
        self.atoms = torch.linspace(-params.atom_vmax, params.atom_vmax, params.n_atoms, device=self.device).repeat(
            self.n_actions, 1)
        on_gpu = self.device.type == "cuda"
        fused_adam = on_gpu and os.environ.get("HB_ADAM_FUSED", "1") != "0"
        self.optimizer = torch.optim.Adam(self.online.parameters(), lr=params.learning_rate, betas=(0.9, 0.999),
                                          eps=3.125e-5, capturable=on_gpu, foreach=(True if on_gpu and not fused_adam else None),
                                          fused=True if fused_adam else None)
        plist = list(self.online.parameters())
        self._flat_grad = torch.zeros(sum(p.numel() for p in plist), dtype=torch.float32, device=self.device)
        off = 0
        for p in plist:
            p.grad = self._flat_grad[off:off + p.numel()].view_as(p)
            off += p.numel()
        self._beta = torch.zeros((), dtype=torch.float32, device=self.device)
        self._beta_host = None
        self.use_graphs = use_graphs
        self._graph1 = self._graph2 = None
        self.train_step = 0
        buf = PriorityBuffer if params.use_priority else ExperienceBuffer
        self.packed = bool(params.packed_obs)
        self.experience = buf(obs_len, self.n_actions, 1, params.experience_buffer_size, device=self.device,
                              seed=params.seed, packed=self.packed)
        self.experience.track_wp = params.n_step > 1
        self.last_obs = (torch.zeros((n_games, bitpack.words_for(obs_len)), dtype=torch.int32, device=self.device) if self.packed
                         else torch.zeros((n_games, obs_len), dtype=torch.int8, device=self.device))
        self.requires_vectorized_observation = lambda: True
        self._gen = torch.Generator(device=self.device).manual_seed(params.seed + 1)
        self._last_loss = None
        self._fused = self.device.type == "cuda" and self.distributional
        self._plain_fast = (self.device.type == "cuda" and not self.distributional and params.compute_dtype == "bfloat16"
                            and len(params.layers) == 1 and params.layers[0] % 256 == 0)
        self._plain_actor = None
        self._eff_cache = None
        self._trg_cache = None
        self._x_act = None
        self._pending = None
        self._disc = params.discount
        self._fl = None
        self._fv = None
        self.use_fused_learner = use_fused_learner
        self.use_mfma_actor = True
        self._draws = 0
        self.first_game_id = 0
        self._is_max_local = self._is_max_global = None
        self.actor_lag = int(params.actor_lag)
        if self.actor_lag and not (self._fused and use_fused_learner and params.use_priority and len(params.layers) == 1):
            raise ValueError("actor_lag=1 needs the HIP fused learner (GPU, C51 head, one hidden layer) with prioritized replay")
        self.force_collective = False
        self._last_coll = False
        self._ar_avg = None
        self._support0 = None
        self._dense_call = None
        self.split_update = bool(self.actor_lag)
        self.two_graphs = False
        self._pending_fills = []
        self.gathered_ev = None
        self.weights_ev = None

    @property
    def last_loss(self):
        if self._fl is not None and self._last_loss is None:
            return self._fl.loss()
        if self._fv is not None and self._last_loss is None:
            return self._fv.loss()
        return self._last_loss

    @last_loss.setter
    def last_loss(self, value):
        self._last_loss = value

    def _unpack(self, observations) -> Tuple[torch.Tensor, torch.Tensor, bool]:
        obs, legal = observations[1]
        on_device = isinstance(obs, torch.Tensor)
        as_dev = lambda x: (x if isinstance(x, torch.Tensor) else torch.as_tensor(np.asarray(x))).to(self.device)
        return as_dev(obs), as_dev(legal), on_device

    def _vec(self, x, dtype):
        if isinstance(x, torch.Tensor):
            return x.to(device=self.device, dtype=dtype)
        return torch.as_tensor(np.asarray(x)).to(device=self.device, dtype=dtype)

    def _uniform(self, n):
        return torch.rand(n, device=self.device, generator=self._gen)

    def _net_input(self, obs):
        return self._obs_int8(obs).to(torch.float32)

    def _obs_int8(self, obs):
        return bitpack.unpack(obs, self.obs_len) if bitpack.is_packed(obs, self.obs_len) else obs

    def _obs_store(self, obs):
        return self.experience.obs_rows(obs)

    def _effective_weights(self):
        if self._fused_learner() is not None:
            return self._fl.eff
        if self._eff_cache is None:
            cd = _DTYPES[self.params.compute_dtype]
            self._eff_cache = [tuple(t.to(cd).contiguous() for t in layer.effective()) for layer in self.online.layers]
        return self._eff_cache

    def _act_plain(self, obs, legal, epsilon):
        from hanabi_hip import _capi as K

        hidden = self.params.layers[0]
        kp = (self.obs_len + 63) // 64 * 64
        pa = self._plain_actor_obj()
        fv = self._fv
        if (fv is not None and fv.cd == torch.bfloat16 and self._graphs_enabled() and obs.is_contiguous()
                and os.environ.get("HB_PLAIN_ACT_GRAPH", "1") != "0"):
            key = (obs.data_ptr(), obs.shape[0], obs.dtype, id(fv), fv.w1cat.data_ptr())
            pg = getattr(pa, "graph", None)
            if pg is not None and pg[0] == key:
                pg[1].replay()
                pa.stale, self._eff_cache = False, True
                return self._plain_select(pg[2], legal, epsilon, obs.shape[0])
            seen = getattr(pa, "graph_seen", None)
            pa.graph_seen = (key, seen[1] + 1) if seen is not None and seen[0] == key else (key, 1)
            if pa.graph_seen[1] >= 3 and getattr(pa, "fv_jobs", None) is not None and pa.h is not None and pa.h.shape[0] == obs.shape[0]:
                n = obs.shape[0]
                packed = obs.dtype == torch.int32
                fn = K.lib().hb_actor_hidden_packed if packed else K.lib().hb_actor_hidden
                qbuf = torch.empty(n, self.n_actions, dtype=torch.float32, device=self.device)

                def forward():
                    st = K.current_stream()
                    K.check(K.lib().hb_actor_pack_weights(pa.fv_jobs, 1, st))
                    pa.w2f.copy_(fv.w2st[0][:, 0:2 * self.n_actions:2])
                    pa.b2f.copy_(fv.b2st[0][0:2 * self.n_actions:2])
                    K.check(fn(K.dptr(obs), n, self.obs_len, K.dptr(pa.w1t), kp, K.dptr(pa.b1), hidden, K.dptr(pa.h), st))
                    torch.addmm(pa.b2f, pa.h.float(), pa.w2f, out=qbuf)

                g = torch.cuda.CUDAGraph()
                with torch.cuda.graph(g, capture_error_mode="thread_local"):
                    forward()
                pa.graph = (key, g, qbuf)
                g.replay()
# ... 238 lines not shown
        self.last_obs = torch.where(first[:, None], self._obs_store(obs), self.last_obs)
        self._dense_call = None

    def add_experience(self, observations, actions, rewards, step_types):
        obs, legal, _ = self._unpack(observations)
        st = self._vec(step_types, torch.int64)
        not_first = st != 0
        idx = torch.nonzero(not_first, as_tuple=False)[:, 0]
        obs8 = self._obs_store(obs)
        if idx.numel():
            self.experience.add_transitions(
                self.last_obs.index_select(0, idx),
                self._vec(actions, torch.int64).index_select(0, idx).reshape(-1, 1),
                self._vec(rewards, torch.float32).index_select(0, idx).reshape(-1, 1),
                obs8.index_select(0, idx),
                legal.index_select(0, idx),
                (st.index_select(0, idx) == 2).reshape(-1, 1))
        self.last_obs = torch.where(not_first[:, None], obs8, self.last_obs)
        self._dense_call = None

    def add_experience_dense(self, observations, actions, rewards, step_types):
        c = self._dense_call
        if c is not None:
            o, l = observations[1]
            try:
                same = (o.data_ptr(), l.data_ptr(), actions.data_ptr(), rewards.data_ptr(), step_types.data_ptr(),
                        self.last_obs.data_ptr(), self.experience._obs_t_buf.data_ptr()) == c[0] and o.shape[0] == c[1]
            except AttributeError:
                same = False
            if same:
                buf, n = self.experience, c[1]
                start = buf.oldest_entry
                if self.params.use_priority:
                    if self.split_update:
                        self._queue_fill(start, n)
                    else:
                        buf.sum_tree.fill_range_dev(start, n, buf._max_priority)
                c[2](*c[3], start, c[4]())
                buf._advance(n)
                return
        obs, legal, _ = self._unpack(observations)
        if self.device.type == "cuda":
            from hanabi_hip import ops

            buf, n = self.experience, obs.shape[0]
            start = buf.oldest_entry
            if self.params.use_priority:
                if self.split_update:
                    self._queue_fill(start, n)
                else:
                    buf.sum_tree.fill_range_dev(start, n, buf._max_priority)
            ins = (self.last_obs, self._obs_store(obs).contiguous(), legal.to(torch.int8).contiguous(),
                   self._vec(actions, torch.int32).contiguous(), self._vec(rewards, torch.float32).contiguous(),
                   self._vec(step_types, torch.int8).contiguous())
            ops.replay_insert(*ins, buf, start)
            buf._advance(n)
            o, l = observations[1]
            if (isinstance(o, torch.Tensor) and all(isinstance(t, torch.Tensor) for t in (l, actions, rewards, step_types))
                    and (ins[1].data_ptr(), ins[2].data_ptr(), ins[3].data_ptr(), ins[4].data_ptr(), ins[5].data_ptr())
                    == (o.data_ptr(), l.data_ptr(), actions.data_ptr(), rewards.data_ptr(), step_types.data_ptr())):
                self._dense_call = ((o.data_ptr(), l.data_ptr(), actions.data_ptr(), rewards.data_ptr(), step_types.data_ptr(),
                                     self.last_obs.data_ptr(), buf._obs_t_buf.data_ptr()), n,
                                    *ops.replay_insert_call(*ins, buf))
            return
        obs8 = self._obs_store(obs)
        st = self._vec(step_types, torch.int64)
        self.experience.add_transitions(self.last_obs, self._vec(actions, torch.int64).reshape(-1, 1),
                                        self._vec(rewards, torch.float32).reshape(-1, 1), obs8, legal,
                                        (st == 2).reshape(-1, 1))
        self.last_obs.copy_(obs8)

    def _sample(self):
        indices, prios = self._sample_indices()
        if self.params.n_step > 1:
            tr, self._disc = self.experience.gather_nstep_dev(indices, self.params.n_step, self.params.discount)
        else:
            tr, self._disc = self.experience.gather_dev(indices), self.params.discount
        return indices, prios, tr

    def update(self):
        self.update_begin()
        self.update_finish()

    def set_two_graphs(self, on=True):
        on = bool(on)
        if on != self.two_graphs:
            assert self._pending is None
            self.two_graphs = on
            self._graph1 = self._graph2 = None
        return on

    def set_split_update(self, on=True):
        on = bool(on) or bool(self.actor_lag)
        if on and not (self._fused and self.use_fused_learner and self.params.use_priority and len(self.params.layers) == 1
                       and not self.params.resample_noise and self._graphs_enabled()):
            return False
        if on != self.split_update:
            assert self._pending is None and not self._pending_fills
            self.split_update = on
            self._graph1 = self._graph2 = None
        return on

    def _queue_fill(self, start, n):
        cap = self.experience.capacity
        pf = self._pending_fills
        if pf and pf[-1][0] + pf[-1][1] == start and pf[-1][1] + n <= cap:
            pf[-1] = (pf[-1][0], pf[-1][1] + n)
        else:
            pf.append((start, n))
        if len(pf) > 1 and sum(x[1] for x in pf) >= cap:
            pf[:] = [(0, cap)]

    def apply_pending_fills(self):
        for start, n in self._pending_fills:
            self.experience.sum_tree.fill_range_dev(start, n, self.experience._max_priority)
        self._pending_fills.clear()

    def _pre_gather(self):
        fl = self._fused_learner()
        fl.sample_and_gather(self.params.seed + 0x51ED270B + 0x9E3779B1 * self.first_game_id)
        if self.gathered_ev is None:
            from hanabi_hip import _capi as K

            self.gathered_ev = K.Event()
        self.gathered_ev.record()

    def update_begin(self):
        assert self._pending is None, "update_finish() of the previous update has not been called"
        if self.split_update:
            self.apply_pending_fills()
        self.experience.sync_size()
        beta = float(self.params.beta_is(self.train_step))
        if beta != self._beta_host:
            self._beta.fill_(beta)
            self._beta_host = beta
        if self._graphs_enabled():
            if self._graph1 is None:
                self._capture_update_graphs()
            if self.split_update:
                self._pre_gather()
            self._graph1.replay()
            part2_args = None
        else:
            if self.split_update:
                self._pre_gather()
            self.last_loss, indices, new_prios = self._update_part1()
            part2_args = (indices, new_prios)
        self._pending = (self._allreduce_gradients(async_op=True), part2_args)

    def update_finish(self):
        if self._pending is None:
            return
        work, part2_args = self._pending
        self._pending = None
        self._finish_allreduce(work)
        if part2_args is None:
            if self._graph2 is not None:
                self._graph2.replay()
            part2_args = (self._g_idx, self._g_prios)
        else:
            self._update_part2(*part2_args)
        self._eff_cache = None
        if self._fl is not None:
            self._fl.weights_updated()
        if self.split_update:
            self._after_optimizer_step(*part2_args)
        if self.train_step % self.params.target_update_period == 0:
            self._sync_target()
        self.train_step += 1

    def _sync_target(self):
# ... 155 lines not shown
        ts = [p.data for p in self.online.parameters()] + list(self.online.buffers())
        ts += [p.data for p in self.target.parameters()] + list(self.target.buffers())
        fl = self._fl
        if fl is not None:
            seen = set()
            for mv in fl.state.values():
                for t in mv:
                    if id(t) not in seen:
                        seen.add(id(t))
                        ts.append(t)
            ts += [fl.step, fl.w1cat, fl.b1cat, fl.w2st, fl.b2st]
        if self.params.use_priority:
            ts += [self.experience._max_priority, self.experience._min_priority]
        return ts

    def _snapshot_learner_state(self):
        snap = dict(tensors=[t.clone() for t in self._learner_state_tensors()], last_loss=self._last_loss,
                    rng=torch.cuda.get_rng_state(self.device), gen=self._gen.get_state())
        xg = getattr(self.experience, "_gen", None)
        if xg is not None:
            snap["xgen"] = xg.get_state()
        if self.params.use_priority:
            snap["tree"] = self.experience.sum_tree.nodes().clone()
        if self._fl is None:
            snap["adam"] = {id(p): {k: (v.clone() if isinstance(v, torch.Tensor) else v) for k, v in st.items()}
                            for p, st in self.optimizer.state.items()}
        return snap

    def _restore_learner_state(self, snap):
        with torch.no_grad():
            for dst, src in zip(self._learner_state_tensors(), snap["tensors"]):
                dst.copy_(src)
            if "tree" in snap:
                self.experience.sum_tree.import_nodes(snap["tree"])
            if "adam" in snap:
                for p, st in self.optimizer.state.items():
                    old = snap["adam"].get(id(p))
                    for k, v in st.items():
                        if isinstance(v, torch.Tensor):
                            v.zero_() if old is None else v.copy_(old[k])
        torch.cuda.set_rng_state(snap["rng"], self.device)
        self._gen.set_state(snap["gen"])
        if "xgen" in snap:
            self.experience._gen.set_state(snap["xgen"])
        self._last_loss = snap["last_loss"]
        self._eff_cache = None
        if self._fv is not None:
            self._fv.refresh_all()
        if self._fl is not None and self._fl.thin:
            self._fl._transpose(0)
            self._fl._transpose(1)
        if self._fl is not None and not self.actor_lag:
            self._fl.actor_stale = True

    def _capture_update_graphs(self):
        cur = torch.cuda.current_stream()
        side = torch.cuda.Stream()
        side.wait_stream(cur)
        self._fused_learner()
        with torch.cuda.stream(side):
            snap = self._snapshot_learner_state()
            for _ in range(3):
                self._update_eager()
            self._restore_learner_state(snap)
        cur.wait_stream(side)
        torch.cuda.synchronize()
        self._graph1, self._graph2 = torch.cuda.CUDAGraph(), torch.cuda.CUDAGraph()
        if not self._collective() and not (self.two_graphs and not self.actor_lag and self.split_update):
            with torch.cuda.graph(self._graph1, capture_error_mode="thread_local"):
                self.last_loss, self._g_idx, self._g_prios = self._update_part1()
                self._update_part2(self._g_idx, self._g_prios)
            self._graph2 = None
            return
        if self._collective_in_graph():
            import torch.distributed as dist

            flat = self._fl.flat_grad if self._fl is not None else self._flat_grad
            with torch.cuda.graph(self._graph1, capture_error_mode="thread_local"):
                self.last_loss, self._g_idx, self._g_prios = self._update_part1()
                dist.all_reduce(flat, op=dist.ReduceOp.AVG, group=self.process_group)
                self._update_part2(self._g_idx, self._g_prios)
            self._graph2 = None
            return
        with torch.cuda.graph(self._graph1, capture_error_mode="thread_local"):
            self.last_loss, self._g_idx, self._g_prios = self._update_part1()
        with torch.cuda.graph(self._graph2, pool=self._graph1.pool(), capture_error_mode="thread_local"):
            self._update_part2(self._g_idx, self._g_prios)

    def _collective_in_graph(self):
        import torch.distributed as dist

        return (os.environ.get("HB_DP_GRAPH_COLLECTIVE") == "1" and self._graphs_enabled() and self._collective()
                and not self.params.global_is_max and dist.get_backend(self.process_group) == "nccl")

    def _dp_world(self):
        import torch.distributed as dist

        if self.process_group is False:
            return 1
        if self.process_group is None and not (dist.is_available() and dist.is_initialized()):
            return 1
        return dist.get_world_size(self.process_group)

    def _collective(self):
        if self._dp_world() > 1:
            return True
        if self.force_collective and self.process_group is not False:
            import torch.distributed as dist

            return dist.is_available() and dist.is_initialized()
        return False

    def _note_local_is_max(self, prios):
        if self.params.global_is_max and self._dp_world() > 1:
            if self._is_max_local is None:
                self._is_max_local = torch.ones(1, dtype=torch.float32, device=self.device)
                self._is_max_global = torch.ones(1, dtype=torch.float32, device=self.device)
            self._is_max_local.copy_(((1.0 / prios).to(torch.float32) ** self._beta).max().reshape(1))

    def _allreduce_gradients(self, async_op=False):
        import torch.distributed as dist

        coll = self._collective()
        if self._fl is not None and self._fl.direct is not None and self._fl.direct != (not coll):
            raise RuntimeError("the process group changed after the FusedLearner was built: its gradient routing "
                               "(direct GEMM outputs vs packed all-reduce bucket) no longer matches the world size")
        if coll and self._graph1 is not None and self._graph2 is None and self._graphs_enabled():
            coll = False
        self._last_coll = coll
        if not coll:
            return None
        flat = self._fl.flat_grad if self._fl is not None else self._flat_grad
        if self.params.global_is_max:
            self._is_max_global.copy_(self._is_max_local)
            dist.all_reduce(self._is_max_global, op=dist.ReduceOp.MAX, group=self.process_group)
            scale = self._is_max_local / self._is_max_global
            flat.mul_(scale)
            if self._fl is not None:
                self._fl.w_is.mul_(scale)
            elif self._last_loss is not None:
                self._last_loss = self._last_loss * scale[0]
        if self._ar_avg is None:
            self._ar_avg = dist.get_backend(self.process_group) == "nccl"
        work = dist.all_reduce(flat, op=dist.ReduceOp.AVG if self._ar_avg else dist.ReduceOp.SUM, group=self.process_group,
                               async_op=True)
        if not async_op:
            work.wait()
        return work

    def _finish_allreduce(self, work):
        if not self._last_coll:
            return
        if work is not None:
            work.wait()
        if not self._ar_avg:
            flat = self._fl.flat_grad if self._fl is not None else self._flat_grad
            flat /= self._dp_world()

    def __repr__(self):
        return f"<rlax_dqn.DQNAgent(params={self.params})>"

    def save_weights(self, path, fname_part):
        torch.save(self.online.state_dict(), os.path.join(path, "rlax_rainbow_" + fname_part + "_online.pkl"))
        torch.save(self.target.state_dict(), os.path.join(path, "rlax_rainbow_" + fname_part + "_target.pkl"))

    def checkpoint_state(self, include_replay=True):
        if self._pending_fills:
            self.apply_pending_fills()
        sd = dict(format="hanabi-agents_amd/agent/1", params=repr(self.params), train_step=self.train_step,
                  draws=self._draws, first_game_id=self.first_game_id, seed=int(self.params.seed),
# ... 93 lines not shown
```

### hanabi-agents_amd/hanabi_hip/_capi.py

```python
import ctypes as C
import os

_HERE = os.path.dirname(os.path.abspath(__file__))
_LIB = None

FLAG_AUTO_RESET, FLAG_RESET_START_NEXT, FLAG_LENIENT_REWARD = 1, 2, 4
STEP_FIRST, STEP_MID, STEP_LAST = 0, 1, 2


class HbError(RuntimeError):
    pass


class HbConfig(C.Structure):

    _fields_ = [(n, C.c_int32) for n in ("players", "colors", "ranks", "hand_size", "max_info", "max_life", "flags")]

    def __repr__(self):
        return "HbConfig(" + ", ".join(f"{n}={getattr(self, n)}" for n, _ in self._fields_) + ")"


GAME_TYPES = {
    "Hanabi-Full": dict(colors=5, ranks=5, hand_size=lambda p: 5 if p < 4 else 4, max_info=8, max_life=3),
    "Hanabi-Full-CardKnowledge": dict(colors=5, ranks=5, hand_size=lambda p: 5 if p < 4 else 4, max_info=8, max_life=3),
# ... 59 lines not shown
    "hb_abi_version": (C.c_int, []),
    "hb_config_validate": (C.c_int, [_CFG]),
    "hb_num_actions": (C.c_int, [_CFG]),
    "hb_obs_len": (C.c_int, [_CFG]),
    "hb_deck_size": (C.c_int, [_CFG]),
    "hb_state_words": (C.c_int, [_CFG]),
    "hb_obs_words": (C.c_int, [_CFG]),
    "hb_env_create": (C.c_int, [_CFG, _I64, _U64, _I64, C.POINTER(_P)]),
    "hb_env_destroy": (C.c_int, [_P]),
    "hb_env_num_games": (_I64, [_P]),
    "hb_env_set_decks": (C.c_int, [_P, _P]),
    "hb_env_reset": (C.c_int, [_P, _P, _I32, _P]),
    "hb_env_observe": (C.c_int, [_P, _P, _P, _P, _P, _P]),
    "hb_env_step": (C.c_int, [_P] + [_P] * 8 + [_P]),
    "hb_env_observe_packed": (C.c_int, [_P, _P, _P, _P, _P, _P, _P]),
    "hb_env_step_packed": (C.c_int, [_P] + [_P] * 9 + [_P]),
    "hb_env_step_select_packed": (C.c_int, [_P, _P, _P, C.c_float, _U64, _U64, _I64, _P] + [_P] * 8 + [_P]),
    "hb_obs_pack": (C.c_int, [_P, _P, _I64, _I32, _P]),
    "hb_obs_unpack": (C.c_int, [_P, _P, _I64, _I32, _P]),
    "hb_env_illegal_count": (C.c_int, [_P, C.POINTER(_I64)]),
    "hb_env_stats": (C.c_int, [_P, C.POINTER(_I64), C.POINTER(_I64)]),
    "hb_env_export_state": (C.c_int, [_P, _P, _P]),
    "hb_env_import_state": (C.c_int, [_P, _P, _P]),
    "hb_env_state": (_P, [_P]),
    "hb_rule_act": (C.c_int, [_CFG, _P, _I64, _I64, C.POINTER(HbRule), _I32, _U64, _U64, _P, _P, _P]),
    "hb_random_legal_actions": (C.c_int, [_P, _I64, _I32, _U64, _U64, _I64, _P, _P]),
    "hb_env_set_games_per_wave": (C.c_int, [_P, _I32]),
    "hb_env_set_async_refill": (C.c_int, [_P, _I32]),
    "hb_env_set_refill_period": (C.c_int, [_P, _I32]),
    "hb_env_set_profile_events": (C.c_int, [_P, _P, _P]),
    "hb_event_create": (C.c_int, [C.POINTER(_P)]),
    "hb_event_destroy": (C.c_int, [_P]),
    "hb_event_record": (C.c_int, [_P, _P]),
    "hb_stream_wait_event": (C.c_int, [_P, _P]),
    "hb_tree_create": (C.c_int, [_I64, C.POINTER(_P)]),
    "hb_tree_destroy": (C.c_int, [_P]),
    "hb_tree_capacity": (_I64, [_P]),
    "hb_tree_nodes": (_P, [_P]),
    "hb_tree_export_nodes": (C.c_int, [_P, _P, _P]),
    "hb_tree_import_nodes": (C.c_int, [_P, _P, _P]),
    "hb_tree_set_lazy_top": (C.c_int, [_P, _I32]),
    "hb_tree_update": (C.c_int, [_P, _P, _P, _I64, _P]),
    "hb_tree_fill_range": (C.c_int, [_P, _I64, _I64, _P, _P]),
    "hb_tree_sample": (C.c_int, [_P, _P, _P, _P, _I64, _P]),
    "hb_tree_get": (C.c_int, [_P, _P, _P, _I64, _P]),
    "hb_tree_total": (C.c_int, [_P, _P, _P]),
    "hb_tree_error_count": (C.c_int, [_P, C.POINTER(_I64)]),
    "hb_per_sample": (C.c_int, [_P, _P, _I64, _I32, _P, _P, _P]),
    "hb_per_sample_philox": (C.c_int, [_P, _U64, _P, _I64, _P, _P, _P]),
    "hb_per_sample_gather": (C.c_int, [_P, _U64, _P, _I64, _P, _P, _P, _P, _P, _P, _P, _I32, _I32, _P, _I32, _I32, _P, _P, _P, _P, _I32,
                                       C.c_float, _I64, _I64, _P, _P]),
    "hb_per_update": (C.c_int, [_P, _P, _P, _I64, _F64, _P, _P, _P]),
    "hb_obs_cast": (C.c_int, [_P, _P, _I32, _I64, _I32, _I32, _P]),
    "hb_policy_act": (C.c_int, [_P, _I32, _P, _P, _I64, _I32, _I32, _I32, C.c_float, _U64, _U64, _I64, _P, _P, _P]),
    "hb_replay_gather": (C.c_int, [_P] * 6 + [_I64, _I32, _P, _I32, _I32, _P, _P, _P, _P, _I32, C.c_float, _I64, _I64, _P, _P]),
    "hb_replay_gather_packed": (C.c_int, [_P] * 6 + [_I64, _I32, _P, _I32, _I32, _P, _P, _P, _P, _I32, C.c_float, _I64, _I64, _P, _P]),
    "hb_c51_loss_grad": (C.c_int, [_P, _P, _I32, _P, _P, _P, _P, _P, _P, _I32, _P, _I64, _I32, _I32, _I32, _P, _P, _P, _P, _P, _P, _P]),
    "hb_c51_loss_sparse": (C.c_int, [_P, _P, _I32, _P, _P, _P, _P, _P, _P, _I32, _P, _I64, _I32, _I32, _I32, _P, _P, _P, _P, _P, _P, _P]),
    "hb_thin_gemm": (C.c_int, [_P, _P, _P, _P, _I64, _I32, _I32, _I32, _I32, _I32, _I32, _I64, _I64, _I64, _I32, _P]),
    "hb_dqn_loss_sparse": (C.c_int, [_P, _P, _I32, _P, _P, _P, _P, _P, _P, _I64, _I32, _I32, _I32, _P, _P, _P, _P, _P, _P]),
    "hb_c51_backward": (C.c_int, [_P, _P, _P, _I32, _P, _I32, _I32, _I64, _I32, _I32, _I32, _P, _P, _P, _I32, _P, _P]),
    "hb_colsum": (C.c_int, [_P, _I32, _I64, _I64, _P, _P]),
    "hb_noisy_adam": (C.c_int, [_P] * 11 + [_P, _P, _I32, _I64, _I32, _I32, C.c_float, C.c_float, C.c_float, C.c_float, _P]),
    "hb_noisy_adam_multi": (C.c_int, [C.POINTER(HbAdamTensor), _I32, _P, C.c_float, _I32, C.c_float, C.c_float, C.c_float, C.c_float, _P]),
    "hb_actor_pack_weights": (C.c_int, [C.POINTER(HbPackJob), _I32, _P]),
    "hb_actor_hidden": (C.c_int, [_P, _I64, _I32, _P, _I32, _P, _I32, _P, _P]),
    "hb_actor_hidden_packed": (C.c_int, [_P, _I64, _I32, _P, _I32, _P, _I32, _P, _P]),
    "hb_actor_q": (C.c_int, [_P, _I64, _I32, _P, _P, _P, _I32, _I32, _P, _P]),
    "hb_policy_select": (C.c_int, [_P, _P, _I64, _I32, C.c_float, _U64, _U64, _I64, _P, _P]),
    "hb_actor_q_select": (C.c_int, [_P, _I64, _I32, _P, _P, _P, _I32, _I32, _P, _P, C.c_float, _U64, _U64, _I64, _P, _P, _P]),
    "hb_actor_act": (C.c_int, [_P, _I32, _P, _I64, _I32, _P, _I32, _P, _I32, _P, _P, _P, _P, _I32, _I32, _P, C.c_float, _U64, _U64, _I64,
                               _P, _P, _P]),
    "hb_actor_fused_supported": (C.c_int, [_I32, _I32, _I32, _I32]),
    "hb_actor_fused_sizes": (C.c_int, [_I32, _I32, _I32, _I32, C.POINTER(_I64), C.POINTER(_I64), C.POINTER(_I32)]),
    "hb_actor_fused_pack": (C.c_int, [_P, _I32, _P, _P, _I32, _P, _I32, _I32, _I32, _I32, _P, _P, _P, _P, _P]),
    "hb_actor_fused_q": (C.c_int, [_P, _I64, _I32, _P, _P, _P, _P, _P, _I32, _I32, _I32, _P, _P]),
    "hb_actor_fused_act": (C.c_int, [_P, _P, _I64, _I32, _P, _P, _P, _P, _P, _I32, _I32, _I32, _P, C.c_float, _U64, _U64, _I64, _P, _P]),
    "hb_actor_fused_columns": (C.c_int, [_I32, C.POINTER(_I32)]),
    "hb_noisy_adam_multi_pack": (C.c_int, [_P, _P, _I32, _P, C.c_float, _I32, C.c_float, C.c_float, C.c_float, C.c_float, _P]),
    "hb_actor_fused_pack_dt": (C.c_int, [_P, _I32, _P, _P, _I32, _P, _I32, _I32, _I32, _I32, _P, _P, _P, _P, _I32, _P]),
    "hb_actor_fused_pack_thin": (C.c_int, [_P, _I32, _P, _P, _I32, _P, _I32, _I32, _I32, _I32, _P, _P, _P, _P, _P, _I32, _P, _I32, _I32, _P]),
    "hb_actor_fused_q_dt": (C.c_int, [_P, _I64, _I32, _P, _P, _P, _P, _P, _I32, _I32, _I32, _P, _I32, _P]),
    "hb_actor_fused_act_dt": (C.c_int, [_P, _P, _I64, _I32, _P, _P, _P, _P, _P, _I32, _I32, _I32, _P, C.c_float, _U64, _U64, _I64, _P, _I32, _P]),
    "hb_chain_run": (C.c_int, [C.POINTER(HbCmd), _I32, C.POINTER(_I64), C.POINTER(_F64)]),
    "hb_eval_counters": (C.c_int, [_CFG]),
    "hb_eval_tally": (C.c_int, [_CFG, _I64, _I32, _I32] + [_P] * 8 + [_P]),
    "hb_relu_bwd_colsum": (C.c_int, [_P, _P, _I64, _I32, _I64, _I64, _P, _P]),
    "hb_replay_insert": (C.c_int, [_P] * 12 + [_I64, _I32, _I32, _I64, _I64, _P]),
}


def lib():
    global _LIB
    if _LIB is None:
        path = library_path()
        if not os.path.exists(path):
            raise HbError(f"{path} is missing: build it with `python -c 'import __graft_entry__ as g; g.build()'` "
                          f"(there is no CPU fallback)")
        L = C.CDLL(path)
        for name, (res, args) in SIGNATURES.items():
            fn = getattr(L, name)
            fn.restype = res
            fn.argtypes = args
        _LIB = L
    return _LIB


def check(rc):
    if rc != 0:
        raise HbError(f"hanabi_hip error {rc}: {lib().hb_last_error().decode()}")


_RAW_STREAM = None


def current_stream():
    global _RAW_STREAM
    import torch

    if _RAW_STREAM is None:
        raw = getattr(torch._C, "_cuda_getCurrentRawStream", None)
        _RAW_STREAM = (lambda: raw(torch._C._cuda_getDevice())) if raw is not None else (
            lambda: torch.cuda.current_stream().cuda_stream)
    return C.c_void_p(_RAW_STREAM())


def dptr(t):
    return None if t is None else C.c_void_p(t.data_ptr())


class Event:

    __slots__ = ("h", "_lib", "recorded")

    def __init__(self):
        self._lib = lib()
        h = C.c_void_p()
        check(self._lib.hb_event_create(C.byref(h)))
        self.h = h
        self.recorded = False

    def record(self, stream=None):
        check(self._lib.hb_event_record(self.h, current_stream() if stream is None else stream))
        self.recorded = True

    def wait(self, stream=None):
        if self.recorded:
            check(self._lib.hb_stream_wait_event(current_stream() if stream is None else stream, self.h))

    def __del__(self):
        try:
            if self.h:
                self._lib.hb_event_destroy(self.h)
        except Exception:
            pass


def set_stream(stream):
    import torch

    torch._C._cuda_setStream(stream_id=stream.stream_id, device_index=stream.device_index, device_type=stream.device_type)
```

### hanabi-agents_amd/hanabi_hip/selfplay.py

```python
import os

import torch

from . import _capi as K


class SelfPlaySession:
    def __init__(self, env, agents, updates_per_step=1, min_replay=None, train_seats=None, overlap_allreduce=None,
                 learner_stream=True, learner_priority=-1, stream_per_agent=None, fuse_select=True, split_update=True,
                 native_chain=True, early_update=True):
        assert len(agents) == env.players, "one agent per seat"
        self.env = env
        self.agents = list(agents)
        self.updates_per_step = int(updates_per_step)
        self.t = 0
        self.last_actions = [torch.zeros(env.n, dtype=torch.int32, device=env.device) for _ in agents]
        self._act_buf = [torch.zeros(env.n, dtype=torch.int32, device=env.device) for _ in agents]
        self.fuse_select = bool(fuse_select) and getattr(env, "packed", False) and env.device.type == "cuda"
        self.min_replay = min_replay
        self.train_seats = set(range(env.players)) if train_seats is None else set(train_seats)
        if overlap_allreduce is None:
            import torch.distributed as dist

            overlap_allreduce = dist.is_available() and dist.is_initialized() and dist.get_world_size() > 1
        self.overlap_allreduce = bool(overlap_allreduce) and len(set(map(id, agents))) == len(agents)
        self.learner_stream = None
        self._stream_factory = None
        if learner_stream and env.device.type == "cuda" and len(set(map(id, agents))) == len(agents) and len(agents) > 1:
            self._stream_factory = learner_stream if callable(learner_stream) and not isinstance(learner_stream, torch.cuda.Stream) else None
            self.learner_stream = (self._stream_factory() if self._stream_factory else
                                   learner_stream if isinstance(learner_stream, torch.cuda.Stream) else
                                   torch.cuda.Stream(device=env.device, priority=learner_priority))
        self._main, self._main_raw = None, -1
        import torch.distributed as dist

        self._dp = dist.is_available() and dist.is_initialized() and dist.get_world_size() > 1
        self._stream_per_agent = True if stream_per_agent is None else bool(stream_per_agent)
        self._lstreams = {}
        self.max_learner_streams = int(os.environ.get("HB_MAX_LEARNER_STREAMS", "2"))
        if self.learner_stream is not None and split_update:
            for a in agents:
                if hasattr(a, "set_split_update"):
                    a.set_split_update(True)
            if stream_per_agent is None and any(getattr(a, "split_update", False) for a in agents):
                self._stream_per_agent = True
        self._update_done = {}
        self._acted_ev, self._done_ev = {}, {}
        self.env_steps = 0
        self.grad_steps = 0
        self._inflight = None
        self._stats0 = env.stats()
        self.native_chain = bool(native_chain) and env.device.type == "cuda"
        self.early_update = (bool(early_update) and self.native_chain and self.learner_stream is not None
                             and os.environ.get("HB_EARLY_UPDATE", "1") != "0")
        if self.early_update:
            for a in agents:
                if hasattr(a, "set_two_graphs") and getattr(a, "split_update", False) and not getattr(a, "actor_lag", 0):
                    a.set_two_graphs(True)
        self._inserted_ev = {}
        self._acted_early = os.environ.get("HB_ACTED_BEFORE_ENV", "1") != "0"
        self.select_in_env_steps = 0
        self._chains = {}
        self.native_steps = 0
        self._evaluators = {}

    def _chain_for(self, seat, agent, train, raw):
        env = self.env
        if not (self.native_chain and train and self.learner_stream is not None and self.fuse_select and self.updates_per_step == 1
                and seat in self.train_seats and self.t >= env.players and getattr(env, "packed", False)):
            return None
        if not (hasattr(agent, "_fl") and getattr(agent, "split_update", False)):
            return None
        fl, p = agent._fl, agent.params
        lag = int(getattr(agent, "actor_lag", 0))
        if (fl is None or fl.actor is None or fl.actor_stale or not p.use_priority or p.resample_noise or not agent.use_mfma_actor
                or agent._graph1 is None or (agent._graph2 is not None) != bool(getattr(agent, "two_graphs", False) and not lag)
                or agent._pending is not None or agent._pending_fills
                or agent._dense_call is None or fl._sg_call is None or agent.gathered_ev is None or agent.weights_ev is None
                or seat not in self._acted_ev or not self._ready(agent) or not fl.actor.takes_fused(env.net_obs)):
            return None
        if agent.train_step % p.target_update_period == 0:
            return None
        buf = agent.experience
        wset = fl.n_packed % 2 if lag else 0
        if lag and (fl.packed_ev[wset] is None or fl.actor._two_stale[wset]):
            return None
        act = fl.actor
        if act.q is None or act.q.shape[0] != env.n:
            return None
        if agent._support0 is None:
            agent._support0 = agent.atoms[0].contiguous()
        ch = self._chains.get((seat, wset))
        ls = self._learner_stream_of(agent)
        key = (raw, ls.cuda_stream, wset, agent._dense_call[0], fl._sg_call[0], fl._sg_call[1], id(agent._graph1), buf.rows_per_insert,
               self.last_actions[seat].data_ptr(), self._act_buf[seat].data_ptr(), agent._g_idx.data_ptr(), agent._g_prios.data_ptr(),
               act.q.data_ptr(), agent._support0.data_ptr())
        if ch is None or ch.key != key:
            now = (env.net_obs.data_ptr(), env.legal.data_ptr(), self.last_actions[seat].data_ptr(), env.agent_reward.data_ptr(),
                   env.agent_step_type.data_ptr(), agent.last_obs.data_ptr(), buf._obs_t_buf.data_ptr())
            if agent._dense_call[0] != now or agent._dense_call[1] != env.n or self.last_actions[seat] is not self._act_buf[seat]:
                return None
            ch = self._chains[(seat, wset)] = _Chain(self, seat, agent, raw, ls.cuda_stream, key, wset)
        return ch

    def _native_step(self, ch, seat, agent, explore):
        env, buf, fl = self.env, agent.experience, agent._fl
        n = env.n
        vi, vf = ch.vi, ch.vf
        start = buf.oldest_entry
        agent._draws += 1
        vi[0], vi[1], vi[2], vi[3] = start, agent._draws, start, n
        vi[4] = 1 if (self._update_done.pop(id(agent), None) is not None and agent.gathered_ev.recorded) else 0
        vi[5] = 1 if ((fl.packed_ev[ch.wset].recorded if ch.lag else agent.weights_ev.recorded)) else 0
        vf[0] = float(agent.params.epsilon(agent.train_step)) if explore else 0.0
        buf._advance(n)
        beta = float(agent.params.beta_is(agent.train_step))
        if buf._synced != (buf.size, buf.oldest_entry) or beta != agent._beta_host:
            K.set_stream(ch.ls)
            try:
                buf.sync_size()
                if beta != agent._beta_host:
                    agent._beta.fill_(beta)
                    agent._beta_host = beta
            finally:
                K.set_stream(self._main)
        K.check(ch.run(ch.cmds, ch.count, vi, vf))
        agent.gathered_ev.recorded = agent.weights_ev.recorded = True
        self._acted_ev[seat].recorded = True
        if ch.lag:
            fl.packed_ev[ch.wset].recorded = True
            fl.n_packed += 1
        env._obs_stale = True
        self.last_actions[seat] = self._act_buf[seat]
        agent._eff_cache = None
        if not ch.lag:
            fl.weights_updated()
        agent.train_step += 1
        self._update_done[id(agent)] = ch.done
        self.env_steps += n
        self.grad_steps += 1
        self.native_steps += 1
        self.t += 1

    def step(self, train=True, explore=True):
        env = self.env
        seat = self.t % env.players
        agent = self.agents[seat]
# ... 166 lines not shown
                    agent_slot=slot, agents=[u.checkpoint_state(include_replay) for u in uniq])

    def load_checkpoint_state(self, sd):
        if sd.get("format") != "hanabi-agents_amd/session/1":
            raise ValueError("not a session checkpoint")
        if sd["games"] != self.env.n or len(sd["agent_slot"]) != len(self.agents):
            raise ValueError("checkpoint was written for a different number of games / seats")
        if (sd["env_seed"], sd["first_game_id"]) != (self.env.seed, self.env.first_game_id):
            raise ValueError("the env's deck seed / first game id differ from the checkpoint's: future deals would diverge")
        self.flush()
        self.env.import_state(sd["env_rows"])
        self.env.observe()
        for dst, src in zip(self.last_actions, sd["last_actions"]):
            dst.copy_(src)
        done = set()
        for a, k in zip(self.agents, sd["agent_slot"]):
            if id(a) not in done:
                a.load_checkpoint_state(sd["agents"][k])
                done.add(id(a))
        self.t, self.env_steps, self.grad_steps = int(sd["t"]), int(sd["env_steps"]), int(sd["grad_steps"])
        ep, sc = self.env.stats()
        self._stats0 = (ep - sd["episodes"], sc - sd["score_sum"])
        self._update_done.clear()
        self._inflight = None

    def save_checkpoint(self, path, include_replay=True):
        torch.save(self.checkpoint_state(include_replay), path)

    def load_checkpoint(self, path):
        self.load_checkpoint_state(torch.load(path, map_location="cpu", weights_only=True))

    @property
    def episodes(self):
        return self.env.stats()[0] - self._stats0[0]

    def mean_score(self):
        ep, sc = self.env.stats()
        ep, sc = ep - self._stats0[0], sc - self._stats0[1]
        return sc / ep if ep else float("nan")


class _Chain:

    def __init__(self, session, seat, agent, raw, lraw, key, wset=0):
        import ctypes as C

        env, buf, fl = session.env, agent.experience, agent._fl
        self.key, self.ls = key, session._learner_stream_of(agent)
        self.wset, self.lag = wset, bool(getattr(agent, "actor_lag", 0))
        cmds = (K.HbCmd * 20)()
        A, Ls = C.c_void_p(raw), C.c_void_p(lraw)
        n_cmd = [0]

        def put(op, stream, ptrs=(), ints=(), floats=(), var=-1, fvar=-1, cond=-1):
            c = cmds[n_cmd[0]]
            n_cmd[0] += 1
            c.op, c.var, c.fvar, c.cond, c.stream = op, var, fvar, cond, stream
            for j, v in enumerate(ptrs):
                c.p[j] = v.value if isinstance(v, C.c_void_p) else v
            for j, v in enumerate(ints):
                c.i[j] = int(v)
            for j, v in enumerate(floats):
                c.f[j] = float(v)

        acted = session._acted_ev[seat]
        done = session._done_ev.get(id(agent))
        if done is None:
            done = session._done_ev[id(agent)] = K.Event()
        self.done = done
        early = session.early_update and not self.lag
        ins = agent._dense_call[3]
        act = fl.actor
        f = act._fset_ptrs[wset]
        if agent._support0 is None:
            agent._support0 = agent.atoms[0].contiguous()
        put(K.CMD_WAIT_EVENT, A, [agent.gathered_ev.h], cond=4)
        put(K.CMD_REPLAY_INSERT, A, ins[:12], ins[12:16], var=0)
        if early:
            inserted = session._inserted_ev.get(seat)
            if inserted is None:
                inserted = session._inserted_ev[seat] = K.Event()
            put(K.CMD_RECORD_EVENT, A, [inserted.h])
        put(K.CMD_WAIT_EVENT, A, [(fl.packed_ev[wset] if self.lag else agent.weights_ev).h], cond=5)
        put(K.CMD_ACTOR_FUSED_ACT, A,
            [env.net_obs.data_ptr(), env.legal.data_ptr(), f[0], f[1], f[2], f[3], agent._support0.data_ptr(), act.q.data_ptr(),
             session._act_buf[seat].data_ptr()],
            [env.n, act.obs_len, act.hidden, act.n_actions, act.n_atoms, agent.params.seed + 0x9E3779B9, agent.first_game_id, act._dt],
            var=1, fvar=0)
        env_args = [env.h, session._act_buf[seat].data_ptr(), env.obs_bits.data_ptr(), None, env.legal.data_ptr(), env.reward.data_ptr(),
                    env.terminal.data_ptr(), env.agent_reward.data_ptr(), env.agent_step_type.data_ptr(), env.score.data_ptr()]
        if session._acted_early:
            put(K.CMD_RECORD_EVENT, A, [acted.h])
            put(K.CMD_ENV_STEP_PACKED, A, env_args)
        else:
            put(K.CMD_ENV_STEP_PACKED, A, env_args)
            put(K.CMD_RECORD_EVENT, A, [acted.h])
        put(K.CMD_WAIT_EVENT, Ls, [(inserted if early else acted).h])
        put(K.CMD_TREE_FILL_RANGE, Ls, [buf.sum_tree.h, buf._max_priority.data_ptr()], var=2)
        g = fl._sg_call[3]
        put(K.CMD_PER_SAMPLE_GATHER, Ls,
            [g[0], g[2], g[4], g[5], g[6], g[7], g[8], g[9], g[10], g[13], g[16], g[17], g[18], g[19], g[24]],
            [g[1], g[3], g[11], g[12], g[14], g[15], g[20], g[22], g[23]], [g[21]])
        put(K.CMD_RECORD_EVENT, Ls, [agent.gathered_ev.h])
        put(K.CMD_GRAPH_LAUNCH, Ls, [agent._graph1.raw_cuda_graph_exec()])
        if early:
            put(K.CMD_WAIT_EVENT, Ls, [acted.h])
        if agent._graph2 is not None:
            put(K.CMD_GRAPH_LAUNCH, Ls, [agent._graph2.raw_cuda_graph_exec()])
        if self.lag:
            (w1, b1), (w2, b2) = fl.eff
            th = fl._thin_out()
            put(K.CMD_ACTOR_FUSED_PACK, Ls, [w1.data_ptr(), b1.data_ptr(), w2.data_ptr(), b2.data_ptr(), f[0], f[1], f[2], f[3]] +
                ([th[0].data_ptr(), th[2].data_ptr()] if th else [0, 0]),
                [w1.stride(0), w2.stride(0), act.obs_len, act.hidden, act.n_actions, act.n_atoms, act._dt] + ([th[1], th[3]] if th else [0, 0]))
            if act.two_kernel:
                jobs = next(j for kk, j in act._jobs.items() if kk[0] == wset and kk[1] == w1.data_ptr())
                self._jobs = jobs
                put(K.CMD_ACTOR_PACK_WEIGHTS, Ls, [C.addressof(jobs)], [2])
            put(K.CMD_RECORD_EVENT, Ls, [fl.packed_ev[wset].h])
        put(K.CMD_RECORD_EVENT, Ls, [agent.weights_ev.h])
        prios = agent._g_prios
        assert prios.dtype == torch.float32 and prios.is_contiguous() and agent._g_idx.dtype == torch.int64
        put(K.CMD_PER_UPDATE, Ls,
            [buf.sum_tree.h, agent._g_idx.data_ptr(), prios.data_ptr(), buf._max_priority.data_ptr(), buf._min_priority.data_ptr()],
            [agent._g_idx.numel()], [buf.alpha])
        self.cmds, self.count = cmds, n_cmd[0]
        self.vi = (C.c_int64 * 8)()
        self.vf = (C.c_double * 2)()
        self.run = K.lib().hb_chain_run
```

### include/hanabi_hip.h

```cpp
#ifndef HANABI_HIP_H
#define HANABI_HIP_H

#include <stdint.h>

#ifdef __cplusplus
extern "C" {
#endif

#define HB_ABI_VERSION 1

#define HB_OK 0
#define HB_ERR_INVALID (-1)
#define HB_ERR_NO_DEVICE (-2)
#define HB_ERR_HIP (-3)
#define HB_ERR_ALIGN (-4)
#define HB_ERR_NOMEM (-5)

const char* hb_last_error(void);
int hb_abi_version(void);

typedef struct hb_config {
  int32_t players;
  int32_t colors;
  int32_t ranks;
// ... 199 lines not shown
typedef struct hb_adam_tensor {
  float *w, *w_mu, *w_sigma;
  const float* noise;
  const void* grad;
  float *m_w, *v_w, *m_mu, *v_mu, *m_sigma, *v_sigma;
  void* eff;
  int64_t n;
  int32_t cols, eff_ld;
  int32_t grad_dtype, grad_ld;
} hb_adam_tensor;
int hb_noisy_adam_multi(const hb_adam_tensor* tensors , int32_t count,
                        const float* step_dev, float step_offset, int32_t eff_dtype, float lr, float beta1, float beta2,
                        float eps, void* stream);

typedef struct hb_adam_pack {
  void* wt;
  void* frag;
  const int32_t* col_map_dev;
  float* bias_f32;
  int32_t wt_ld, frag_kind;
} hb_adam_pack;
int hb_noisy_adam_multi_pack(const hb_adam_tensor* tensors, const hb_adam_pack* packs, int32_t count, const float* step_dev,
                             float step_offset, int32_t eff_dtype, float lr, float beta1, float beta2, float eps, void* stream);

int hb_relu_bwd_colsum(void* dy_dev, const void* act_dev, int64_t act_ld , int32_t dtype,
                       int64_t rows, int64_t cols, float* out_dev, void* stream);

typedef struct hb_pack_job {
  const void* w;
  const void* bias;
  void* wt;
  float* bias_out;
  int32_t k_rows, n_cols, w_ld, group_cols, k_pad;
} hb_pack_job;
int hb_actor_pack_weights(const hb_pack_job* jobs , int32_t count ,
                          void* stream);
int hb_actor_hidden(const int8_t* obs_dev, int64_t n_rows, int32_t obs_len, const void* w1t_dev, int32_t k_pad,
                    const float* b1_dev, int32_t hidden, void* h_dev, void* stream);
int hb_actor_hidden_packed(const uint32_t* obs_bits_dev, int64_t n_rows, int32_t obs_len, const void* w1t_dev, int32_t k_pad,
                           const float* b1_dev, int32_t hidden, void* h_dev, void* stream);
int hb_actor_q(const void* h_dev, int64_t n_rows, int32_t hidden, const void* w2t_dev, const float* b2_dev,
               const float* support_dev, int32_t n_actions, int32_t n_atoms, float* q_dev, void* stream);
int hb_policy_select(const float* q_dev, const int8_t* legal_dev, int64_t n_games, int32_t n_actions, float epsilon,
                     uint64_t seed, uint64_t draw, int64_t first_game_id, int32_t* actions_dev, void* stream);

int hb_actor_q_select(const void* h_dev, int64_t n_rows, int32_t hidden, const void* w2t_dev, const float* b2_dev,
                      const float* support_dev, int32_t n_actions, int32_t n_atoms, float* q_dev, const int8_t* legal_dev,
                      float epsilon, uint64_t seed, uint64_t draw, int64_t first_game_id, int32_t* actions_dev,
                      uint32_t* tickets_dev, void* stream);

int hb_actor_act(const void* obs_dev, int32_t obs_is_packed, const int8_t* legal_dev, int64_t n_rows, int32_t obs_len,
                 const void* w1t_dev, int32_t k_pad, const float* b1_dev, int32_t hidden, void* h_dev, const void* w2t_dev,
                 const float* b2_dev, const float* support_dev, int32_t n_actions, int32_t n_atoms, float* q_dev, float epsilon,
                 uint64_t seed, uint64_t draw, int64_t first_game_id, int32_t* actions_dev, uint32_t* tickets_dev, void* stream);

int hb_actor_fused_supported(int32_t obs_len, int32_t hidden, int32_t n_actions, int32_t n_atoms);
int hb_actor_fused_sizes(int32_t obs_len, int32_t hidden, int32_t n_actions, int32_t n_atoms, int64_t* w1f_bytes,
                         int64_t* w2f_bytes, int32_t* b2f_floats);
int hb_actor_fused_pack(const void* w1_dev, int32_t w1_ld, const void* b1_dev, const void* w2_dev, int32_t w2_ld,
                        const void* b2_dev, int32_t obs_len, int32_t hidden, int32_t n_actions, int32_t n_atoms, void* w1f_dev,
                        float* b1f_dev, void* w2f_dev, float* b2f_dev, void* stream);
int hb_actor_fused_q(const uint32_t* obs_bits_dev, int64_t n_rows, int32_t obs_len, const void* w1f_dev, const float* b1f_dev,
                     const void* w2f_dev, const float* b2f_dev, const float* support_dev, int32_t hidden, int32_t n_actions,
                     int32_t n_atoms, float* q_dev, void* stream);
int hb_actor_fused_act(const uint32_t* obs_bits_dev, const int8_t* legal_dev, int64_t n_rows, int32_t obs_len, const void* w1f_dev,
                       const float* b1f_dev, const void* w2f_dev, const float* b2f_dev, const float* support_dev, int32_t hidden,
                       int32_t n_actions, int32_t n_atoms, float* q_dev, float epsilon, uint64_t seed, uint64_t draw,
                       int64_t first_game_id, int32_t* actions_dev, void* stream);
int hb_actor_fused_columns(int32_t n_actions, int32_t* phys_of_logit_host);
int hb_actor_fused_pack_dt(const void* w1_dev, int32_t w1_ld, const void* b1_dev, const void* w2_dev, int32_t w2_ld,
                           const void* b2_dev, int32_t obs_len, int32_t hidden, int32_t n_actions, int32_t n_atoms, void* w1f_dev,
                           float* b1f_dev, void* w2f_dev, float* b2f_dev, int32_t dtype, void* stream);
int hb_actor_fused_pack_thin(const void* w1_dev, int32_t w1_ld, const void* b1_dev, const void* w2_dev, int32_t w2_ld,
                             const void* b2_dev, int32_t obs_len, int32_t hidden, int32_t n_actions, int32_t n_atoms,
                             void* w1f_dev, float* b1f_dev, void* w2f_dev, float* b2f_dev, void* w1t_dev, int32_t w1t_ld,
                             void* w2t_dev, int32_t w2t_ld, int32_t dtype, void* stream);
int hb_actor_fused_q_dt(const uint32_t* obs_bits_dev, int64_t n_rows, int32_t obs_len, const void* w1f_dev, const float* b1f_dev,
                        const void* w2f_dev, const float* b2f_dev, const float* support_dev, int32_t hidden, int32_t n_actions,
                        int32_t n_atoms, float* q_dev, int32_t dtype, void* stream);
int hb_actor_fused_act_dt(const uint32_t* obs_bits_dev, const int8_t* legal_dev, int64_t n_rows, int32_t obs_len,
                          const void* w1f_dev, const float* b1f_dev, const void* w2f_dev, const float* b2f_dev,
                          const float* support_dev, int32_t hidden, int32_t n_actions, int32_t n_atoms, float* q_dev, float epsilon,
                          uint64_t seed, uint64_t draw, int64_t first_game_id, int32_t* actions_dev, int32_t dtype, void* stream);

int hb_eval_counters(const hb_config* cfg);
int hb_eval_tally(const hb_config* cfg, int64_t n_games, int32_t seat, int32_t turn, const int32_t* actions_dev,
                  const float* reward_dev, const int8_t* terminal_dev, const int8_t* score_dev, uint8_t* done_dev,
                  int8_t* final_score_dev, int16_t* length_dev, int64_t* counters_dev, void* stream);

enum {
  HB_CMD_WAIT_EVENT = 1,
  HB_CMD_RECORD_EVENT = 2,
  HB_CMD_REPLAY_INSERT = 3,
  HB_CMD_ACTOR_FUSED_ACT = 4,
  HB_CMD_ENV_STEP_PACKED = 5,
  HB_CMD_TREE_FILL_RANGE = 6,
  HB_CMD_PER_SAMPLE_GATHER = 7,
  HB_CMD_GRAPH_LAUNCH = 8,
  HB_CMD_PER_UPDATE = 9,
  HB_CMD_ACTOR_FUSED_PACK = 10,
  HB_CMD_ACTOR_PACK_WEIGHTS = 11
};
typedef struct hb_cmd {
  int32_t op, var, fvar, cond;
  void* stream;
  void* p[16];
  int64_t i[10];
  double f[2];
} hb_cmd;
int hb_chain_run(const hb_cmd* cmds, int32_t count, const int64_t* vars_i, const double* vars_f);

#ifdef __cplusplus
}
#endif
#endif
```

Baseline: 300.2 million.

## Fuse env step into actor kernel tail and run Adam early in update graph

Adds a combined actor+env kernel. After action selection, each block keeps its picked actions in LDS and its first waves run the env step for those games directly, so there is no separate env-step launch and the actions are not read back from global memory. The env kernel body is factored into a reusable wave-level step, and the env args are read from the kernarg segment. The self-play chain uses the fused command when the config is supported, and optionally moves the Adam update into the first update graph. The risk is that reads of obs/legal and the in-place env writes now race within a single kernel, and the fused kernel's larger register/LDS footprint may lower occupancy.

```diff
diff --git a/hanabi-agents_amd/csrc/actor_fused.hip b/hanabi-agents_amd/csrc/actor_fused.hip
--- a/hanabi-agents_amd/csrc/actor_fused.hip
+++ b/hanabi-agents_amd/csrc/actor_fused.hip
@@ -3,6 +3,7 @@
 #include <hip/hip_fp16.h>
 
 #include <cstdint>
+#include <type_traits>
 
 #include "../../include/hanabi_hip.h"
 #include "common.hpp"
@@ -112,8 +113,8 @@
 }
 __device__ __forceinline__ float exp2_fast(float x) { return __builtin_amdgcn_exp2f(x); }
 
-template <bool F16>
-__global__ __launch_bounds__(FNT) void actor_fused_kernel(const FusedArgs a) {
+template <bool F16, class K, int EG>
+__device__ __forceinline__ void actor_fused_body(const FusedArgs& a) {
   __shared__ __attribute__((aligned(16))) unsigned char lds[LDS_TOTAL];
   const int tid = threadIdx.x, lane = tid & 63;
   const int wave = __builtin_amdgcn_readfirstlane(tid >> 6);
@@ -460,9 +461,41 @@
         pick = __ffsll(static_cast<long long>(pool)) - 1;
       }
       a.actions[g] = pick;
+      if constexpr (!std::is_void_v<K>) reinterpret_cast<int*>(lds + H_BYTES)[tid] = pick;
+    }
+  }
+  if constexpr (!std::is_void_v<K>) {
+    constexpr int ENV_WORDS = hb::env_lds_words<K, EG>();
+    static_assert((FM / EG) * ENV_WORDS * 4 <= H_BYTES && FM / EG <= FNT / 64, "env tail: the LDS slices must fit in H");
+    __syncthreads();
+    if (wave < FM / EG) {
+#if defined(__HIP_DEVICE_COMPILE__)
+      typedef const __attribute__((address_space(4))) unsigned char KargByte;
+      typedef const __attribute__((address_space(4))) hb::EnvArgs KargEnv;
+      auto kargs = __builtin_amdgcn_kernarg_segment_ptr();
+      asm volatile("" : "+s"(kargs));
+      constexpr size_t ENV_OFF = (sizeof(FusedArgs) + alignof(hb::EnvArgs) - 1) / alignof(hb::EnvArgs) * alignof(hb::EnvArgs);
+      KargEnv& env = *(KargEnv*)((KargByte*)kargs + ENV_OFF);
+#else
+      const hb::EnvArgs env{};
+#endif
+      const long long g0 = row0 + EG * wave;
+      const int uid = lane < EG ? reinterpret_cast<const int*>(lds + H_BYTES)[EG * wave + lane] : 0;
+      hb::env_wave_step<K, EG>(env, g0, lane, reinterpret_cast<uint32_t*>(lds) + wave * ENV_WORDS, uid, g0 / EG);
     }
   }
   HB_FSTAMP_REAL(15);
+}
+
+template <bool F16>
+__global__ __launch_bounds__(FNT) void actor_fused_kernel(const FusedArgs a) {
+  actor_fused_body<F16, void, 16>(a);
+}
+
+template <bool F16, class K, int EG>
+__global__ __launch_bounds__(FNT) void actor_env_fused_kernel(const FusedArgs a, const hb::EnvArgs env) {
+  (void)env;
+  actor_fused_body<F16, K, EG>(a);
 }
 
 struct PackArgs {
@@ -650,16 +683,18 @@
 }
 #endif
 
-static int fused_launch(const uint32_t* obs_bits_dev, int64_t n_rows, int32_t obs_len, const void* w1f_dev, const float* b1f_dev,
-                        const void* w2f_dev, const float* b2f_dev, const float* support_dev, int32_t hidden, int32_t n_actions,
-                        int32_t n_atoms, float* q_dev, unsigned long long* stamps_dev, const FusedSelect* sel, int32_t dtype, void* stream) {
+static int fused_args(const uint32_t* obs_bits_dev, int64_t n_rows, int32_t obs_len, const void* w1f_dev, const float* b1f_dev,
+                      const void* w2f_dev, const float* b2f_dev, const float* support_dev, int32_t hidden, int32_t n_actions,
+                      int32_t n_atoms, float* q_dev, unsigned long long* stamps_dev, const FusedSelect* sel, int32_t dtype, FusedArgs& a,
+                      bool* launch) {
+  *launch = false;
   if (dtype != 1 && dtype != 2) return fail(HB_ERR_INVALID, "dtype must be 1 (bf16) or 2 (f16)");
   if (!obs_bits_dev || !w1f_dev || !b1f_dev || !w2f_dev || !b2f_dev || !support_dev || !q_dev) return fail(HB_ERR_INVALID, "null argument");
   if (!hb_actor_fused_supported(obs_len, hidden, n_actions, n_atoms)) return fail(HB_ERR_INVALID, "shape not covered by the fused actor kernel");
   if (n_rows <= 0) return HB_OK;
   if (!aligned16(w1f_dev) || !aligned16(w2f_dev) || !aligned16(b1f_dev) || !aligned16(b2f_dev))
     return fail(HB_ERR_ALIGN, "w1f / w2f / b1f / b2f must be 16-byte aligned");
-  FusedArgs a{};
+  a = FusedArgs{};
   a.obs = obs_bits_dev; a.m = n_rows; a.words = (obs_len + 31) / 32; a.s1 = 2 * ((obs_len + 63) / 64);
   a.w1f = static_cast<const uint4*>(w1f_dev); a.b1 = b1f_dev; a.w2f = static_cast<const uint4*>(w2f_dev); a.b2 = b2f_dev;
   a.support = support_dev; a.q = q_dev; a.n_actions = n_actions; a.n_pass = passes_for(n_actions);
@@ -668,6 +703,19 @@
     a.legal = sel->legal; a.actions = sel->actions; a.epsilon = sel->epsilon; a.seed = sel->seed; a.draw = sel->draw;
     a.first_gid = sel->first_gid;
   }
+  *launch = true;
+  return HB_OK;
+}
+
+static int fused_launch(const uint32_t* obs_bits_dev, int64_t n_rows, int32_t obs_len, const void* w1f_dev, const float* b1f_dev,
+                        const void* w2f_dev, const float* b2f_dev, const float* support_dev, int32_t hidden, int32_t n_actions,
+                        int32_t n_atoms, float* q_dev, unsigned long long* stamps_dev, const FusedSelect* sel, int32_t dtype, void* stream) {
+  FusedArgs a;
+  bool go = false;
+  if (int rc = fused_args(obs_bits_dev, n_rows, obs_len, w1f_dev, b1f_dev, w2f_dev, b2f_dev, support_dev, hidden, n_actions, n_atoms, q_dev,
+                          stamps_dev, sel, dtype, a, &go))
+    return rc;
+  if (!go) return HB_OK;
   const dim3 grid(static_cast<unsigned>((n_rows + FM - 1) / FM));
   if (dtype == 2) hipLaunchKernelGGL(actor_fused_kernel<true>, grid, dim3(FNT), 0, static_cast<hipStream_t>(stream), a);
   else hipLaunchKernelGGL(actor_fused_kernel<false>, grid, dim3(FNT), 0, static_cast<hipStream_t>(stream), a);
@@ -676,3 +724,60 @@
 }
 
 }
+
+namespace {
+
+using ActEnvFull2 = hb::Cfg<2, 5, 5, 5, 8, 3>;
+using ActEnvFull5 = hb::Cfg<5, 5, 5, 4, 8, 3>;
+constexpr int ENV_EG = 16;
+
+template <class K>
+static bool is_cfg(const hb::EnvVariant& v) {
+  return v.P == K::P && v.C == K::C && v.R == K::R && v.H == K::H && v.INFO == K::INFO && v.LIFE == K::LIFE;
+}
+
+template <bool F16, class K>
+static void launch_act_env(const FusedArgs& a, const hb::EnvArgs& env, dim3 grid, hipStream_t stream) {
+  if (env.ev_start && env.ev_stop)
+    hipExtLaunchKernelGGL((actor_env_fused_kernel<F16, K, ENV_EG>), grid, dim3(FNT), 0, stream, env.ev_start, env.ev_stop, 0, a, env);
+  else
+    hipLaunchKernelGGL((actor_env_fused_kernel<F16, K, ENV_EG>), grid, dim3(FNT), 0, stream, a, env);
+}
+
+}
+
+namespace hb {
+
+bool actor_env_fused_supported(const EnvVariant& v) { return is_cfg<ActEnvFull2>(v) || is_cfg<ActEnvFull5>(v); }
+
+int actor_env_fused_launch(const uint32_t* obs_bits_dev, const int8_t* legal_dev, int64_t n_rows, int32_t obs_len, const void* w1f_dev,
+                           const float* b1f_dev, const void* w2f_dev, const float* b2f_dev, const float* support_dev, int32_t hidden,
+                           int32_t n_actions, int32_t n_atoms, float* q_dev, float epsilon, uint64_t seed, uint64_t draw,
+                           int64_t first_game_id, int32_t* actions_dev, int32_t dtype, const EnvArgs& env, const EnvVariant& var,
+                           void* stream) {
+  if (!legal_dev || !actions_dev) return fail(HB_ERR_INVALID, "null argument");
+  if (!actor_env_fused_supported(var)) return fail(HB_ERR_INVALID, "no fused policy + env kernel for this game configuration");
+  if (n_rows != env.n) return fail(HB_ERR_INVALID, "n_rows (%lld) must equal the env's game count (%lld)", static_cast<long long>(n_rows), env.n);
+  if (n_actions != var.n_actions || obs_len != var.obs_len) return fail(HB_ERR_INVALID, "actor shape does not match the env");
+  const FusedSelect sel{legal_dev, actions_dev, epsilon, seed, draw, first_game_id};
+  FusedArgs a;
+  bool go = false;
+  if (int rc = fused_args(obs_bits_dev, n_rows, obs_len, w1f_dev, b1f_dev, w2f_dev, b2f_dev, support_dev, hidden, n_actions, n_atoms, q_dev,
+                          nullptr, &sel, dtype, a, &go))
+    return rc;
+  if (!go) return HB_OK;
+  const dim3 grid(static_cast<unsigned>((n_rows + FM - 1) / FM));
+  const hipStream_t st = static_cast<hipStream_t>(stream);
+  const bool f16 = dtype == 2;
+  if (is_cfg<ActEnvFull2>(var)) {
+    if (f16) launch_act_env<true, ActEnvFull2>(a, env, grid, st);
+    else launch_act_env<false, ActEnvFull2>(a, env, grid, st);
+  } else {
+    if (f16) launch_act_env<true, ActEnvFull5>(a, env, grid, st);
+    else launch_act_env<false, ActEnvFull5>(a, env, grid, st);
+  }
+  HB_HIP(hipGetLastError());
+  return HB_OK;
+}
+
+}
diff --git a/hanabi-agents_amd/csrc/chain.hip b/hanabi-agents_amd/csrc/chain.hip
--- a/hanabi-agents_amd/csrc/chain.hip
+++ b/hanabi-agents_amd/csrc/chain.hip
@@ -36,6 +36,17 @@
         break;
       case HB_CMD_ACTOR_FUSED_ACT:
         if (!vi || !vf) return fail(HB_ERR_INVALID, "command %d: hb_actor_fused_act needs its draw and epsilon variables", k);
+        if (c.p[9]) {
+          rc = hb_actor_fused_act_step(static_cast<hb_env*>(c.p[9]), static_cast<const uint32_t*>(c.p[0]), static_cast<const int8_t*>(c.p[1]),
+                                       c.i[0], static_cast<int32_t>(c.i[1]), c.p[2], static_cast<const float*>(c.p[3]), c.p[4],
+                                       static_cast<const float*>(c.p[5]), static_cast<const float*>(c.p[6]), static_cast<int32_t>(c.i[2]),
+                                       static_cast<int32_t>(c.i[3]), static_cast<int32_t>(c.i[4]), static_cast<float*>(c.p[7]),
+                                       static_cast<float>(vf[0]), static_cast<uint64_t>(c.i[5]), static_cast<uint64_t>(vi[0]), c.i[6],
+                                       static_cast<int32_t*>(c.p[8]), c.i[7] == 2 ? 2 : 1, static_cast<uint32_t*>(c.p[0]),
+                                       static_cast<int8_t*>(c.p[1]), static_cast<float*>(c.p[10]), static_cast<int8_t*>(c.p[11]),
+                                       static_cast<float*>(c.p[12]), static_cast<int8_t*>(c.p[13]), static_cast<int8_t*>(c.p[14]), c.stream);
+          break;
+        }
         rc = hb_actor_fused_act_dt(static_cast<const uint32_t*>(c.p[0]), static_cast<const int8_t*>(c.p[1]), c.i[0],
                                    static_cast<int32_t>(c.i[1]), c.p[2], static_cast<const float*>(c.p[3]), c.p[4],
                                    static_cast<const float*>(c.p[5]), static_cast<const float*>(c.p[6]), static_cast<int32_t>(c.i[2]),
diff --git a/hanabi-agents_amd/csrc/env_api.hip b/hanabi-agents_amd/csrc/env_api.hip
--- a/hanabi-agents_amd/csrc/env_api.hip
+++ b/hanabi-agents_amd/csrc/env_api.hip
@@ -229,7 +229,7 @@
   return HB_OK;
 }
 
-static int launch(hb_env* e, hb::EnvArgs& a, void* stream) {
+static void prepare(hb_env* e, hb::EnvArgs& a) {
   a.state = e->state;
   a.decks = e->decks;
   a.next_deck = e->next_deck;
@@ -246,6 +246,10 @@
   }
   a.ev_start = e->ev_start;
   a.ev_stop = e->ev_stop;
+}
+
+static int launch(hb_env* e, hb::EnvArgs& a, void* stream) {
+  prepare(e, a);
   const int gpw = e->gpw ? e->gpw : ((a.obs_bits && !a.obs && e->n >= 32768) ? 32 : 16);
   hb::LaunchFn fn = gpw == 8 ? e->var->g8 : (gpw == 16 ? e->var->g16 : (gpw == 32 ? e->var->g32 : e->var->g64));
   fn(a, static_cast<hipStream_t>(stream));
@@ -380,6 +384,34 @@
   if (int rc = launch(e, a, stream)) return rc;
   return refill_async(e, stream);
 }
+
+int hb_actor_fused_act_step(hb_env* e, const uint32_t* obs_bits_dev, const int8_t* legal_dev, int64_t n_rows, int32_t obs_len,
+                            const void* w1f_dev, const float* b1f_dev, const void* w2f_dev, const float* b2f_dev, const float* support_dev,
+                            int32_t hidden, int32_t n_actions, int32_t n_atoms, float* q_dev, float epsilon, uint64_t seed, uint64_t draw,
+                            int64_t first_game_id, int32_t* actions_dev, int32_t dtype, uint32_t* obs_bits_out_dev, int8_t* legal_out_dev,
+                            float* reward_dev, int8_t* terminal_dev, float* agent_reward_dev, int8_t* agent_step_type_dev,
+                            int8_t* score_dev, void* stream) {
+  if (!e) return fail(HB_ERR_INVALID, "null env");
+  if (int rc = check_out_packed(obs_bits_out_dev, nullptr, legal_out_dev)) return rc;
+  hb::EnvArgs a{};
+  a.mode = hb::MODE_STEP;
+  a.obs_bits = obs_bits_out_dev;
+  a.legal = legal_out_dev;
+  a.reward = reward_dev;
+  a.terminal = terminal_dev;
+  a.agent_reward = agent_reward_dev;
+  a.agent_step_type = agent_step_type_dev;
+  a.score = score_dev;
+  prepare(e, a);
+  if (int rc = join_refill(e, stream)) return rc;
+  if (int rc = hb::actor_env_fused_launch(obs_bits_dev, legal_dev, n_rows, obs_len, w1f_dev, b1f_dev, w2f_dev, b2f_dev, support_dev, hidden,
+                                          n_actions, n_atoms, q_dev, epsilon, seed, draw, first_game_id, actions_dev, dtype, a, *e->var,
+                                          stream))
+    return rc;
+  return refill_async(e, stream);
+}
+
+int hb_actor_fused_step_supported(const hb_env* e) { return e && hb::actor_env_fused_supported(*e->var) ? 1 : 0; }
 
 #ifdef HB_STAMPS
 int hb_env_step_stamped(hb_env* e, const int32_t* actions_dev, int8_t* obs_dev, int8_t* legal_dev,
diff --git a/hanabi-agents_amd/csrc/env_kernel.hpp b/hanabi-agents_amd/csrc/env_kernel.hpp
--- a/hanabi-agents_amd/csrc/env_kernel.hpp
+++ b/hanabi-agents_amd/csrc/env_kernel.hpp
@@ -50,12 +50,12 @@
     unsigned long long hb_t_;                                                                        \
     asm volatile("s_memtime %0\n\ts_waitcnt lgkmcnt(0)" : "=s"(hb_t_)::"memory");                    \
     __builtin_amdgcn_sched_barrier(0);                                                               \
-    if (a.stamps && lane == 0) a.stamps[(static_cast<long long>(blockIdx.x) * 4 + wave) * 12 + (slot)] = hb_t_; \
+    if (a.stamps && lane == 0) a.stamps[wslot * 12 + (slot)] = hb_t_; \
   } while (0)
 #define HB_STAMP_REAL(slot)                                                                          \
   do {                                                                                               \
     if (a.stamps && lane == 0)                                                                       \
-      a.stamps[(static_cast<long long>(blockIdx.x) * 4 + wave) * 12 + (slot)] = __builtin_amdgcn_s_memrealtime(); \
+      a.stamps[wslot * 12 + (slot)] = __builtin_amdgcn_s_memrealtime(); \
   } while (0)
 #else
 #define HB_STAMP(slot) do { } while (0)
@@ -273,18 +273,15 @@
 }
 
 template <class K, int G>
-__global__ __launch_bounds__(256) void env_kernel(const EnvArgs a) {
+constexpr int env_lds_words() { return G * (K::SWP + K::NWP + K::LW); }
+
+template <class K, int G>
+__device__ __forceinline__ void env_wave_step(const EnvArgs& a, long long g0, int lane, uint32_t* const srow, int uid_in,
+                                              long long wslot) {
   constexpr int P = K::P, C = K::C, R = K::R, H = K::H;
   constexpr int LPG = 1;
-  constexpr int PER_WAVE = G * (K::SWP + K::NWP + K::LW);
-  __shared__ uint32_t lds[4 * PER_WAVE];
-
-  const int lane = threadIdx.x & 63;
-  const int wave = threadIdx.x >> 6;
-  uint32_t* const srow = lds + wave * PER_WAVE;
   uint32_t* const obits = srow + G * K::SWP;
   uint32_t* const lbits = obits + G * K::NWP;
-  const long long g0 = (static_cast<long long>(blockIdx.x) * 4 + wave) * G;
   const long long left = a.n - g0;
   const int nvalid = left <= 0 ? 0 : (left < G ? static_cast<int>(left) : G);
   const int mode = a.mode;
@@ -293,12 +290,10 @@
 
   const bool active = lane < nvalid && lane < G;
   const long long gi = g0 + lane;
-  int uid_in = 0;
   bool mask_in = true;
   uint4 nd[4] = {make_uint4(0u, 0u, 0u, 0u), make_uint4(0u, 0u, 0u, 0u), make_uint4(0u, 0u, 0u, 0u), make_uint4(0u, 0u, 0u, 0u)};
   const uint4* const ndp = reinterpret_cast<const uint4*>(a.next_deck + gi * NEXT_DECK_BYTES);
   if (active) {
-    if (mode == MODE_STEP) uid_in = a.sel_q ? select_action<K::A>(a, gi) : a.actions[gi];
     if (mode == MODE_RESET && a.mask) mask_in = a.mask[gi] != 0;
     if ((mode == MODE_RESET && mask_in) || (mode == MODE_STEP && (a.flags & 0x100))) {
       nd[0] = ndp[0]; nd[1] = ndp[1]; nd[2] = ndp[2]; nd[3] = ndp[3];
@@ -640,7 +635,7 @@
       int sc = out_term ? out_score : 0;
       for (int o = 32; o > 0; o >>= 1) sc += __shfl_xor(sc, o);
       if (lane == 0) {
-        unsigned long long* slot = a.stats + 2 * (static_cast<long long>(blockIdx.x) * 4 + wave);
+        unsigned long long* slot = a.stats + 2 * wslot;
         atomicAdd(slot, static_cast<unsigned long long>(__popcll(ended)));
         atomicAdd(slot + 1, static_cast<unsigned long long>(sc));
       }
@@ -675,6 +670,18 @@
   }
   HB_STAMP(9);
   HB_STAMP_REAL(11);
+}
+
+template <class K, int G>
+__global__ __launch_bounds__(256) void env_kernel(const EnvArgs a) {
+  __shared__ uint32_t lds[4 * env_lds_words<K, G>()];
+  const int lane = threadIdx.x & 63;
+  const int wave = threadIdx.x >> 6;
+  const long long wslot = static_cast<long long>(blockIdx.x) * 4 + wave;
+  const long long g0 = wslot * G;
+  int uid_in = 0;
+  if (a.mode == MODE_STEP && lane < G && g0 + lane < a.n) uid_in = a.sel_q ? select_action<K::A>(a, g0 + lane) : a.actions[g0 + lane];
+  env_wave_step<K, G>(a, g0, lane, lds + wave * env_lds_words<K, G>(), uid_in, wslot);
 }
 
 template <class K>
@@ -747,4 +754,11 @@
                     &launch_env<K, 8>, &launch_env<K, 16>, &launch_env<K, 32>, &launch_env<K, 64>, &launch_refill<K>};
 }
 
-}
+bool actor_env_fused_supported(const EnvVariant& v);
+int actor_env_fused_launch(const uint32_t* obs_bits_dev, const int8_t* legal_dev, int64_t n_rows, int32_t obs_len, const void* w1f_dev,
+                           const float* b1f_dev, const void* w2f_dev, const float* b2f_dev, const float* support_dev, int32_t hidden,
+                           int32_t n_actions, int32_t n_atoms, float* q_dev, float epsilon, uint64_t seed, uint64_t draw,
+                           int64_t first_game_id, int32_t* actions_dev, int32_t dtype, const EnvArgs& env, const EnvVariant& var,
+                           void* stream);
+
+}
diff --git a/hanabi-agents_amd/hanabi_agents/rlax_dqn/fused_learner.py b/hanabi-agents_amd/hanabi_agents/rlax_dqn/fused_learner.py
--- a/hanabi-agents_amd/hanabi_agents/rlax_dqn/fused_learner.py
+++ b/hanabi-agents_amd/hanabi_agents/rlax_dqn/fused_learner.py
@@ -302,15 +302,19 @@
             self._pack_tab = tab
         return self._pack_tab
 
-    def part2(self):
+    def part2(self, opt=True, pack=True):
         p = self.agent.params
         if self.adam_pack:
+            assert opt and pack, "hb_noisy_adam_multi_pack: the optimizer step and the copies are one launch"
             K.check(K.lib().hb_noisy_adam_multi_pack(self._adam_table(), self._pack_table(), 4, K.dptr(self.step), 0.0, _DT[self.cd],
                                                      float(p.learning_rate), 0.9, 0.999, 3.125e-5, K.current_stream()))
             self._packed_in_part2 = True
             return
-        K.check(K.lib().hb_noisy_adam_multi(self._adam_table(), 4, K.dptr(self.step), 0.0, _DT[self.cd],
-                                            float(p.learning_rate), 0.9, 0.999, 3.125e-5, K.current_stream()))
+        if opt:
+            K.check(K.lib().hb_noisy_adam_multi(self._adam_table(), 4, K.dptr(self.step), 0.0, _DT[self.cd],
+                                                float(p.learning_rate), 0.9, 0.999, 3.125e-5, K.current_stream()))
+        if not pack:
+            return
         self._packed_in_part2 = False
         if self.actor is not None and not self.lag:
             (w1, b1), (w2, b2) = self.eff
diff --git a/hanabi-agents_amd/hanabi_agents/rlax_dqn/rlax_rainbow.py b/hanabi-agents_amd/hanabi_agents/rlax_dqn/rlax_rainbow.py
--- a/hanabi-agents_amd/hanabi_agents/rlax_dqn/rlax_rainbow.py
+++ b/hanabi-agents_amd/hanabi_agents/rlax_dqn/rlax_rainbow.py
@@ -161,6 +161,7 @@
         self._dense_call = None
         self.split_update = bool(self.actor_lag)
         self.two_graphs = False
+        self.adam_first = False
         self._pending_fills = []
         self.gathered_ev = None
         self.weights_ev = None
@@ -565,11 +566,11 @@
         self.update_begin()
         self.update_finish()
 
-    def set_two_graphs(self, on=True):
-        on = bool(on)
-        if on != self.two_graphs:
+    def set_two_graphs(self, on=True, adam_first=False):
+        on, adam_first = bool(on), bool(adam_first)
+        if on != self.two_graphs or adam_first != self.adam_first:
             assert self._pending is None
-            self.two_graphs = on
+            self.two_graphs, self.adam_first = on, adam_first
             self._graph1 = self._graph2 = None
         return on
 
@@ -891,10 +892,17 @@
                 self._update_part2(self._g_idx, self._g_prios)
             self._graph2 = None
             return
+        adam_early = (self._fl is not None and not self._fl.adam_pack and not self._collective() and self.two_graphs and self.adam_first
+                      and self._fl.actor is not None and self._fl.actor.fused and self.use_mfma_actor)
         with torch.cuda.graph(self._graph1, capture_error_mode="thread_local"):
             self.last_loss, self._g_idx, self._g_prios = self._update_part1()
+            if adam_early:
+                self._fl.part2(pack=False)
         with torch.cuda.graph(self._graph2, pool=self._graph1.pool(), capture_error_mode="thread_local"):
-            self._update_part2(self._g_idx, self._g_prios)
+            if adam_early:
+                self._fl.part2(opt=False)
+            else:
+                self._update_part2(self._g_idx, self._g_prios)
 
     def _collective_in_graph(self):
         import torch.distributed as dist
diff --git a/hanabi-agents_amd/hanabi_hip/_capi.py b/hanabi-agents_amd/hanabi_hip/_capi.py
--- a/hanabi-agents_amd/hanabi_hip/_capi.py
+++ b/hanabi-agents_amd/hanabi_hip/_capi.py
@@ -165,6 +165,9 @@
     "hb_actor_fused_pack_thin": (C.c_int, [_P, _I32, _P, _P, _I32, _P, _I32, _I32, _I32, _I32, _P, _P, _P, _P, _P, _I32, _P, _I32, _I32, _P]),
     "hb_actor_fused_q_dt": (C.c_int, [_P, _I64, _I32, _P, _P, _P, _P, _P, _I32, _I32, _I32, _P, _I32, _P]),
     "hb_actor_fused_act_dt": (C.c_int, [_P, _P, _I64, _I32, _P, _P, _P, _P, _P, _I32, _I32, _I32, _P, C.c_float, _U64, _U64, _I64, _P, _I32, _P]),
+    "hb_actor_fused_act_step": (C.c_int, [_P, _P, _P, _I64, _I32, _P, _P, _P, _P, _P, _I32, _I32, _I32, _P, C.c_float, _U64, _U64, _I64, _P,
+                                          _I32] + [_P] * 7 + [_P]),
+    "hb_actor_fused_step_supported": (C.c_int, [_P]),
     "hb_chain_run": (C.c_int, [C.POINTER(HbCmd), _I32, C.POINTER(_I64), C.POINTER(_F64)]),
     "hb_eval_counters": (C.c_int, [_CFG]),
     "hb_eval_tally": (C.c_int, [_CFG, _I64, _I32, _I32] + [_P] * 8 + [_P]),
diff --git a/hanabi-agents_amd/hanabi_hip/selfplay.py b/hanabi-agents_amd/hanabi_hip/selfplay.py
--- a/hanabi-agents_amd/hanabi_hip/selfplay.py
+++ b/hanabi-agents_amd/hanabi_hip/selfplay.py
@@ -53,16 +53,21 @@
         self.native_chain = bool(native_chain) and env.device.type == "cuda"
         self.early_update = (bool(early_update) and self.native_chain and self.learner_stream is not None
                              and os.environ.get("HB_EARLY_UPDATE", "1") != "0")
+        self.fuse_env_step = (os.environ.get("HB_FUSED_ENV_STEP", "1") != "0" and getattr(env, "packed", False)
+                              and env.device.type == "cuda" and self._fused_step_ok())
         if self.early_update:
             for a in agents:
                 if hasattr(a, "set_two_graphs") and getattr(a, "split_update", False) and not getattr(a, "actor_lag", 0):
-                    a.set_two_graphs(True)
+                    a.set_two_graphs(True, adam_first=self.fuse_env_step)
         self._inserted_ev = {}
         self._acted_early = os.environ.get("HB_ACTED_BEFORE_ENV", "1") != "0"
         self.select_in_env_steps = 0
         self._chains = {}
         self.native_steps = 0
         self._evaluators = {}
+
+    def _fused_step_ok(self):
+        return bool(K.lib().hb_actor_fused_step_supported(self.env.h))
 
     def _chain_for(self, seat, agent, train, raw):
         env = self.env
@@ -395,19 +400,26 @@
                 inserted = session._inserted_ev[seat] = K.Event()
             put(K.CMD_RECORD_EVENT, A, [inserted.h])
         put(K.CMD_WAIT_EVENT, A, [(fl.packed_ev[wset] if self.lag else agent.weights_ev).h], cond=5)
-        put(K.CMD_ACTOR_FUSED_ACT, A,
-            [env.net_obs.data_ptr(), env.legal.data_ptr(), f[0], f[1], f[2], f[3], agent._support0.data_ptr(), act.q.data_ptr(),
-             session._act_buf[seat].data_ptr()],
-            [env.n, act.obs_len, act.hidden, act.n_actions, act.n_atoms, agent.params.seed + 0x9E3779B9, agent.first_game_id, act._dt],
-            var=1, fvar=0)
-        env_args = [env.h, session._act_buf[seat].data_ptr(), env.obs_bits.data_ptr(), None, env.legal.data_ptr(), env.reward.data_ptr(),
-                    env.terminal.data_ptr(), env.agent_reward.data_ptr(), env.agent_step_type.data_ptr(), env.score.data_ptr()]
-        if session._acted_early:
+        act_ints = [env.n, act.obs_len, act.hidden, act.n_actions, act.n_atoms, agent.params.seed + 0x9E3779B9, agent.first_game_id, act._dt]
+        self.fused_step = session.fuse_env_step and early and env.net_obs.data_ptr() == env.obs_bits.data_ptr()
+        act_ptrs = [env.net_obs.data_ptr(), env.legal.data_ptr(), f[0], f[1], f[2], f[3], agent._support0.data_ptr(), act.q.data_ptr(),
+                    session._act_buf[seat].data_ptr()]
+        if self.fused_step:
+            put(K.CMD_ACTOR_FUSED_ACT, A,
+                act_ptrs + [env.h, env.reward.data_ptr(), env.terminal.data_ptr(), env.agent_reward.data_ptr(), env.agent_step_type.data_ptr(),
+                            env.score.data_ptr()],
+                act_ints, var=1, fvar=0)
             put(K.CMD_RECORD_EVENT, A, [acted.h])
-            put(K.CMD_ENV_STEP_PACKED, A, env_args)
         else:
-            put(K.CMD_ENV_STEP_PACKED, A, env_args)
-            put(K.CMD_RECORD_EVENT, A, [acted.h])
+            put(K.CMD_ACTOR_FUSED_ACT, A, act_ptrs, act_ints, var=1, fvar=0)
+            env_args = [env.h, session._act_buf[seat].data_ptr(), env.obs_bits.data_ptr(), None, env.legal.data_ptr(), env.reward.data_ptr(),
+                        env.terminal.data_ptr(), env.agent_reward.data_ptr(), env.agent_step_type.data_ptr(), env.score.data_ptr()]
+            if session._acted_early:
+                put(K.CMD_RECORD_EVENT, A, [acted.h])
+                put(K.CMD_ENV_STEP_PACKED, A, env_args)
+            else:
+                put(K.CMD_ENV_STEP_PACKED, A, env_args)
+                put(K.CMD_RECORD_EVENT, A, [acted.h])
         put(K.CMD_WAIT_EVENT, Ls, [(inserted if early else acted).h])
         put(K.CMD_TREE_FILL_RANGE, Ls, [buf.sum_tree.h, buf._max_priority.data_ptr()], var=2)
         g = fl._sg_call[3]
diff --git a/include/hanabi_hip.h b/include/hanabi_hip.h
--- a/include/hanabi_hip.h
+++ b/include/hanabi_hip.h
@@ -305,6 +305,13 @@
                           const void* w1f_dev, const float* b1f_dev, const void* w2f_dev, const float* b2f_dev,
                           const float* support_dev, int32_t hidden, int32_t n_actions, int32_t n_atoms, float* q_dev, float epsilon,
                           uint64_t seed, uint64_t draw, int64_t first_game_id, int32_t* actions_dev, int32_t dtype, void* stream);
+int hb_actor_fused_act_step(hb_env* env, const uint32_t* obs_bits_dev, const int8_t* legal_dev, int64_t n_rows, int32_t obs_len,
+                            const void* w1f_dev, const float* b1f_dev, const void* w2f_dev, const float* b2f_dev,
+                            const float* support_dev, int32_t hidden, int32_t n_actions, int32_t n_atoms, float* q_dev, float epsilon,
+                            uint64_t seed, uint64_t draw, int64_t first_game_id, int32_t* actions_dev, int32_t dtype,
+                            uint32_t* obs_bits_out_dev, int8_t* legal_out_dev, float* reward_dev, int8_t* terminal_dev,
+                            float* agent_reward_dev, int8_t* agent_step_type_dev, int8_t* score_dev, void* stream);
+int hb_actor_fused_step_supported(const hb_env* env);
 
 int hb_eval_counters(const hb_config* cfg);
 int hb_eval_tally(const hb_config* cfg, int64_t n_games, int32_t seat, int32_t turn, const int32_t* actions_dev,
```

Measured after the change: 309.9 million (median of 6 runs). +3.2%, better.
